# waveygang/wfmash

Measured on AMD Instinct MI355X. Metric: aligned bases/sec (whole node) + CIGAR-identical rate vs CPU ref, higher is better.
Workload: dtype int32; 1 GPU; C3: 64 synthetic 5%-divergence 50kb segment pairs per GPU, WFA-only (BiWFA gap-affine-2p 5,8,2,24,1; mappings pre-supplied); pairs_per_gpu=64, pairs_total=64, parallelism=records sharded over 1 GPU(s)

## Files before the change

include/wfmash_host.h:

```cpp
#ifndef WFMASH_HOST_H_
#define WFMASH_HOST_H_

#include <stdint.h>
#include "wfmash_hip.h"

#ifdef __cplusplus
extern "C" {
#endif

typedef struct {
  int32_t  mismatch, gap_open1, gap_ext1, gap_open2, gap_ext2;
  float    min_identity;
  uint64_t min_alignment_length;
  float    min_block_identity;
  uint64_t target_padding;
  uint64_t query_padding;
  uint64_t wflign_max_len_minor;
  int32_t  disable_chain_patching;
  int32_t  sam_format;
  int32_t  emit_md_tag;
  int32_t  no_seq_in_sam;
  int32_t  threads;
  int32_t  resident_sequences;
} wfmh_align_params_t;

typedef struct {
  uint64_t records;
  uint64_t aligned_bp;
  uint64_t written;
  uint64_t skipped;
  uint64_t cells;
  double   ms_gpu;
  double   ms_total;
  double   ms_rows;
  double   ms_fetch;
  double   ms_wflign;
  double   ms_text;
  uint64_t batches;
  uint64_t cells_tile;
  uint64_t tile_launches;
  double   ms_tile;
  double   ms_tags;
  uint64_t records_resident;
  uint64_t lazy_fetches;
} wfmh_align_summary_t;

void wfmh_align_default_params(wfmh_align_params_t* p);

int wfmh_align_paf(wfm_handle_t* h, const char* target_fasta, const char* query_fasta,
                   const char* mapping_paf, const char* out_paf,
                   const wfmh_align_params_t* params, wfmh_align_summary_t* summary);

int wfmh_align_paf_multi(wfm_handle_t* const* handles, int n, const char* target_fasta, const char* query_fasta,
                         const char* mapping_paf, const char* out_paf,
                         const wfmh_align_params_t* params, wfmh_align_summary_t* summary);

void wfmh_set_verify(int on);
int  wfmh_verify_counts(uint64_t out[4]);
int  wfmh_verify_paf(wfm_handle_t* h, const char* target_fasta, const char* query_fasta, const char* aligned_paf, uint64_t out[4]);
char* wfmh_test_verify_parse(const char* line);

void wfmh_set_verify_optimal(int on, uint64_t max_cells);
int  wfmh_verify_optimal_counts(uint64_t out[4]);

void wfmh_set_left_align(int on);
int  wfmh_left_align_counts(uint64_t out[4]);

void wfmh_set_cs(int form);
int  wfmh_cs_counts(uint64_t out[4]);

void wfmh_set_variants(const char* path_or_null);
int  wfmh_variants_counts(uint64_t out[4]);

void wfmh_set_coverage(const char* path_or_null);
int  wfmh_coverage_counts(uint64_t out[4]);
int  wfmh_coverage_paf(wfm_handle_t* h, const char* target_fasta, const char* aligned_paf, const char* out_path, uint64_t out[4]);
char* wfmh_test_coverage_bedgraph(const char* const* names, const uint64_t* lengths, int n_seq, const uint64_t* starts, const uint32_t* depths,
                                  int64_t n_iv);

void wfmh_set_lift(const char* bed_path_or_null, const char* out_path_or_null);
int  wfmh_lift_counts(uint64_t out[4]);
int  wfmh_lift_paf(wfm_handle_t* h, const char* target_fasta, const char* aligned_paf, const char* bed_path, const char* out_path, uint64_t out[4]);
void wfmh_set_chain(const char* path_or_null, int swap);
int  wfmh_chain_counts(uint64_t out[4]);
int  wfmh_chain_paf(wfm_handle_t* h, const char* target_fasta, const char* aligned_paf, const char* out_path, int swap, uint64_t out[4]);
void wfmh_set_maf(const char* path_or_null, uint32_t split);
int  wfmh_maf_counts(uint64_t out[4]);
int  wfmh_maf_paf(wfm_handle_t* h, const char* target_fasta, const char* query_fasta_or_null, const char* aligned_paf, const char* out_path, uint32_t split,
                  uint64_t out[4]);
char* wfmh_test_chain_lines(const char* spec, int swap, uint32_t* flags_out);
void wfmh_set_chain_net(const char* path_or_null);
int  wfmh_chain_net_counts(uint64_t out[4]);
int  wfmh_chain_net_paf(wfm_handle_t* h, const char* target_fasta, const char* aligned_paf, const char* out_path, uint64_t out[4]);
char* wfmh_test_chain_net_lines(const char* spec);
void wfmh_set_transitive(const char* bed_path_or_null, const char* out_path_or_null, uint32_t depth);
int  wfmh_transitive_counts(uint64_t out[4]);
int  wfmh_transitive_paf(wfm_handle_t* h, const char* target_fasta, const char* query_fasta_or_null, const char* aligned_paf, const char* bed_path,
                         const char* out_path, uint32_t depth, uint64_t out[4]);
char* wfmh_test_transitive_lines(const char* const* tnames, const uint64_t* tlengths, int n_t, const char* const* qnames, const uint64_t* qlengths,
                                 int n_q, const char* bed, const char* spec);

void wfmh_set_pav(const char* bed_path_or_null, uint64_t window, const char* out_path_or_null);
int  wfmh_pav_counts(uint64_t out[4]);
int  wfmh_pav_paf(wfm_handle_t* h, const char* target_fasta, const char* query_fasta_or_null, const char* aligned_paf, const char* bed_path_or_null,
                  uint64_t window, const char* out_path, uint64_t out[4]);
void wfmh_set_genotypes(const char* path_or_null);
int  wfmh_genotypes_counts(uint64_t out[4]);
char* wfmh_test_genotype_text(const char* version, const char* const* tnames, const uint64_t* lengths, int n_t, const char* const* keys, int n_groups,
                              const uint64_t* sites, size_t n_sites, const char* alleles, const char* gt);

char* wfmh_test_pav_text(const char* const* names, int n_q, const char* const* tnames, const uint64_t* lengths, int n_t, uint64_t window);

char* wfmh_test_lift_lines(const char* const* names, const uint64_t* lengths, int n_seq, const char* bed, const char* spec);

char* wfmh_test_cigar(const char* fn, const char* a, const char* b, const char* query, const char* target,
                      long long i0, long long i1);
void  wfmh_free(char* p);
void  wfmh_test_subwindow(int64_t win_start, int64_t win_end, int rev, int64_t a, int64_t b, int64_t* out_start, int64_t* out_end);
int wfmh_test_rows(const int32_t* q, int64_t n, int64_t* out);
int wfmh_test_tile_plan(const int32_t* jobs, int64_t n, const int32_t* rules, int32_t* per_block, int32_t* tasks, int64_t tasks_cap, int64_t* scalars);
int wfmh_test_p2_plan(const int32_t* cand, int64_t n, int64_t i0, int rows, int rows_bm, unsigned long long budget, int threads, int core, int64_t* geo,
                      int32_t* tasks, int64_t tasks_cap, int64_t* scalars);
int wfmh_test_base_plan(int op, const int32_t* in, int64_t n, int32_t* out);
int wfmh_test_reuse_plan(int op, const int64_t* in, int64_t n, int64_t* out);
int wfmh_test_planned_meet(const int64_t* in, int64_t n, int64_t* out);
int wfmh_test_tile_plan_dirs(const int32_t* jobs, int64_t n, const int32_t* rules, const uint8_t* dirs, int32_t* per_block, int32_t* tasks, int64_t tasks_cap,
                             int64_t* scalars);
int wfmh_test_tile_interior(const int32_t* q, int64_t n, int32_t* out);
int wfmh_test_tile_lean_waves(const int32_t* in, int64_t* out);
int wfmh_test_opt_band(const int64_t* in, int64_t* out);
int64_t wfmh_test_winnow(const char* seq, int64_t len, int k, int w, int s, int32_t seq_id,
                         const uint64_t* hash, const int8_t* strand, wfm_minmer_t* out, int64_t cap);

int64_t wfmh_test_winnow_chunked(const char* seq, int64_t len, int k, int w, int s, int32_t seq_id,
                                 const uint64_t* hash, const int8_t* strand, int64_t chunk_len,
                                 wfm_minmer_t* out, int64_t cap, int* replays);

int64_t wfmh_test_winnow_thinned(const char* seq, int64_t len, int k, int w, int s, int32_t seq_id,
                                 const uint64_t* hash, const int8_t* strand, double c_factor, int64_t chunk_len,
                                 wfm_minmer_t* out, int64_t cap, uint32_t* kept_pos, int64_t cap_kept,
                                 int64_t* n_kept, int* replays);

void wfmh_test_sort_records(wfm_minmer_t* recs, int64_t n, int threads);
int wfmh_test_packed_lce(const uint8_t* buf_p, int64_t n_p, int64_t start_p, const uint8_t* buf_t, int64_t n_t, int64_t start_t, int v, int h, int maxn);
int wfmh_test_is_acgt(const uint8_t* seq, int64_t n);

int64_t wfmh_test_winnow_model(const char* seq, int64_t len, int k, int w, int s, int32_t seq_id, const uint64_t* hash,
                               const int8_t* strand, double c_factor, int64_t chunk_len, wfm_minmer_t* out, int64_t cap,
                               uint32_t* why);

void wfmh_test_sortlike_model(wfm_minmer_t* recs, int64_t n);

int64_t wfmh_test_finish_records(const wfm_minmer_t* raw, int64_t n, int w, wfm_minmer_t* out, int64_t cap);


typedef struct {
  int32_t  kmer_size;
  int64_t  window_length;
  int64_t  block_length;
  int64_t  chain_gap;
  uint64_t max_mapping_length;
  float    percentage_identity;
  int32_t  sketch_size;
  int32_t  filter_mode;
  uint32_t num_mappings_for_segment;
  uint32_t num_mappings_for_scaffold;
  int32_t  drop_rand;
  int32_t  split;
  int32_t  merge_mappings;
  int32_t  skip_self;
  int32_t  skip_prefix;
  int32_t  lower_triangular;
  char     prefix_delim;
  int32_t  filter_length_mismatches;
  uint64_t sparsity_hash_threshold;
  double   overlap_threshold;
  double   scaffold_overlap_threshold;
  int64_t  scaffold_max_deviation;
  int64_t  scaffold_gap;
  int64_t  scaffold_min_length;
  int32_t  legacy_output;
  int32_t  minimum_hits;
  double   max_kmer_freq;
  int64_t  index_by_size;
  float    kmer_complexity_threshold;
  int32_t  stage1_topani_filter;
  int32_t  stage2_full_scan;
  float    ani_diff, ani_diff_conf;
  double   hg_numerator;
  int32_t  threads;
  int32_t  auto_pct_identity;
  int32_t  ani_percentile;
  float    ani_adjustment;
  const char* target_prefix;
  const char* target_list;
  const char* query_prefix;
  const char* query_list;
  const char* index_file;
  int32_t  write_index;
  int32_t  pad_;
  const char* scaffold_out;
  int32_t  streaming_minhash;
} wfmh_map_params_t;

void wfmh_map_default_params(wfmh_map_params_t* p);

typedef struct {
  uint64_t targets, queries, subsets;
  uint64_t target_bp, query_bp;
  uint64_t index_windows;
  uint64_t fragments;
  uint64_t l2_mappings;
  uint64_t written;
  float    percentage_identity;
  int32_t  sketch_size;
  double   ms_index, ms_map, ms_filter, ms_total;
  double   ms_replicate;
  double   ms_identity;
  double   ms_wall;
  int32_t  index_parts;
  int32_t  pad_;
  double   ms_index_sketch;
  double   ms_index_merge;
} wfmh_map_summary_t;

int wfmh_map(wfm_handle_t* h, const char* target_fasta, const char* query_fasta, const char* out_paf,
             const wfmh_map_params_t* params, wfmh_map_summary_t* summary);

int wfmh_map_multi(wfm_handle_t* const* handles, int n, const char* target_fasta, const char* query_fasta, const char* out_paf,
                   const wfmh_map_params_t* params, wfmh_map_summary_t* summary);

typedef struct {
  char*    query_group;
  char*    target_group;
  uint64_t query_hashes, target_hashes, shared;
  double   jaccard, ani;
} wfmh_ani_row_t;
int  wfmh_ani_matrix(wfm_handle_t* const* handles, int n, const char* target_fasta, const char* query_fasta,
                     const wfmh_map_params_t* params, const char* out_tsv);
int  wfmh_ani_matrix_rows(wfm_handle_t* const* handles, int n, const char* target_fasta, const char* query_fasta,
                          const wfmh_map_params_t* params, wfmh_ani_row_t** rows, int64_t* n_rows);
void wfmh_free_ani_rows(wfmh_ani_row_t* rows, int64_t n_rows);
void wfmh_set_ani_matrix(const char* out_tsv);
char* wfmh_test_ani_tsv(const char* const* query_groups, const char* const* target_groups, const uint64_t* query_hashes,
                        const uint64_t* target_hashes, const uint64_t* shared, int64_t n);

int wfmh_test_deal(const int64_t* lengths, int64_t n, int n_parts, int32_t* out_part);

int wfmh_test_map_plan(int op, const int64_t* in, int64_t n, int64_t* out);

int wfmh_seed_paf(const char* target_fasta, const char* query_fasta, const char* seeds_paf, const char* out_paf,
                  const wfmh_map_params_t* params, wfmh_map_summary_t* summary);

char* wfmh_test_filter(const char* stage, const wfm_mapping_t* maps, int64_t n, const char* fasta,
                       const char* query_name, const wfmh_map_params_t* prm);
char* wfmh_test_filter_ordered(const char* stage, const wfm_mapping_t* maps, int64_t n, const uint32_t* orig, const char* fasta,
                               const char* query_name, const wfmh_map_params_t* prm);

char* wfmh_test_fasta(const char* path, const char* name, int64_t start, int64_t end_inclusive, int whole);

void wfmh_release_sequences(void);

char* wfmh_test_fasta_shared(const char* path, const char* name);

int wfmh_test_index_file(const char* op, const char* fasta, char prefix_delim, const char* in_path, const char* out_path);

#ifdef __cplusplus
}
#endif
#endif
```

wfmash_amd/capi.py:

```python
import ctypes as C
import os

import numpy as np

_HERE = os.path.dirname(os.path.abspath(__file__))
LIB_PATH = os.environ.get("WFM_LIB_PATH") or os.path.join(_HERE, "libwfmash_hip.so")

WFM_MODE_END2END_BIWFA = 0
WFM_MODE_ENDSFREE = 1
WFM_MODE_END2END_UNI = 2
WFM_MODE_MASK = 0xff
WFM_MODE_SCORE_ONLY = 0x100
WFM_MODE_SCORE_LIMIT = 0x200
WFM_ST_MAX_SCORE = -100

DEFAULT_PEN = (5, 8, 2, 24, 1)
WFM_PF_ROOT_AGAIN, WFM_PF_JOB_AGAIN, WFM_PF_BASE_RETRY, WFM_PF_BASE_RETRY2, WFM_PF_BYTE_KERNEL, WFM_PF_P2_ROUNDS, WFM_PF_RING_KERNEL, WFM_PF_BASE_TILES = 1, 2, 4, 8, 16, 32, 64, 128
WFM_PF_RING_GROWN = 256
TILE_COUNTERS = ("jobs", "exact_ends", "fine_reruns", "gap_reruns", "ring3", "blocks_coarse", "blocks_fine", "left_band",
                 "reuse_resumed", "reuse_fallbacks", "reuse_keeps", "reuse_touched", "reuse_fell_other", "planned_ends",
                 "p2_exact", "p2_exact_misses")

EXPORTS = [
    "wfm_create", "wfm_destroy", "wfm_last_error", "wfm_device_name",
# ... 1566 lines not shown
        ident = np.ascontiguousarray(p2["ident_table"], dtype=np.uint16)
        cut = np.ascontiguousarray(p2["cutoff_j"], dtype=np.float64)
        P = MapParams()
        P.kmer_size = k
        P.kmer_complexity_threshold = kc_threshold
        P.l1 = L1Params(p1["window_length"], p1["sketch_size"], p1["min_hits_cached"], p1["cached_segment_length"],
                        int(p1["skip_self"]), int(p1["skip_prefix"]), int(p1["lower_triangular"]), int(p1["stage1_topani"]),
                        int(p1["stage2_full_scan"]), len(rg), rg.ctypes.data, mh.ctypes.data, sc.ctypes.data, len(sc), 0)
        P.l2 = L2Params(p2["window_length"], p2["sketch_size"], int(p2["stage1_topani"]), 0, keep.ctypes.data, ident.ctypes.data,
                        cut.ctypes.data)
        buf = np.frombuffer(seq, dtype=np.uint8)
        f = self._L.wfm_map_fragments
        f.restype = C.c_int64
        f.argtypes = [C.c_void_p, C.c_void_p, C.c_void_p, C.c_int64, C.c_void_p, C.c_void_p, C.c_int64, C.POINTER(MapParams),
                      C.c_void_p, C.c_void_p, C.c_int64]
        cap = 1 << 16
        while True:
            out = np.zeros(cap, dtype=MAPPING_DTYPE)
            frag = np.zeros(cap, dtype=np.int32)
            n = f(self._p, index._p, buf.ctypes.data, len(seq), off.ctypes.data, sid.ctypes.data, len(off), C.byref(P),
                  out.ctypes.data, frag.ctypes.data, cap)
            if n < 0:
                raise WfmError(f"wfm_map_fragments failed ({n}): {self.last_error()}")
            if n <= cap:
                return out[:n], frag[:n]
            cap = int(n)

    def minhash_sketch(self, seq: bytes, k: int = 21, sketch_size: int = 4096):
        out = np.zeros(sketch_size, dtype=np.uint64)
        buf = np.frombuffer(seq, dtype=np.uint8)
        f = self._L.wfm_minhash_sketch
        f.restype = C.c_int64
        f.argtypes = [C.c_void_p, C.c_void_p, C.c_int64, C.c_int, C.c_int, C.c_void_p]
        n = f(self._p, buf.ctypes.data, len(seq), k, sketch_size, out.ctypes.data)
        if n < 0:
            raise WfmError(f"wfm_minhash_sketch failed ({n}): {self.last_error()}")
        return out[:n]

    def sketch_intersections(self, sketches, rows=None, cols=None, offsets=None):
        n = len(sketches)
        parts = [np.ascontiguousarray(s, dtype=np.uint64) for s in sketches]
        hashes = np.concatenate(parts) if parts else np.zeros(0, dtype=np.uint64)
        if offsets is None:
            offsets = np.concatenate([[0], np.cumsum([len(p) for p in parts], dtype=np.int64)])
        offs = np.ascontiguousarray(offsets, dtype=np.int64)
        if len(offs) != n + 1:
            raise ValueError("one offset per sketch and one more")
        r = np.ascontiguousarray(np.arange(n) if rows is None else rows, dtype=np.int32)
        c = np.ascontiguousarray(np.arange(n) if cols is None else cols, dtype=np.int32)
        out = np.zeros((len(r), len(c)), dtype=np.uint32)
        f = self._L.wfm_sketch_intersections
        f.restype = C.c_int
        f.argtypes = [C.c_void_p, C.c_void_p, C.c_void_p, C.c_int64, C.c_void_p, C.c_int64, C.c_void_p, C.c_int64, C.c_void_p]
        rc = f(self._p, hashes.ctypes.data, offs.ctypes.data, n, r.ctypes.data, len(r), c.ctypes.data, len(c), out.ctypes.data)
        if rc != 0:
            raise WfmError(f"wfm_sketch_intersections failed ({rc}): {self.last_error()}")
        return out

    def map_l2(self, index, qsketch, qcount, q_len, q_kc, s, cands, params):
        nfrag = len(qcount)
        q = np.ascontiguousarray(qsketch, dtype=MINMER_DTYPE)
        qc = np.ascontiguousarray(qcount, dtype=np.int32)
        ql = np.ascontiguousarray(q_len, dtype=np.int32)
        kc = np.ascontiguousarray(q_kc, dtype=np.uint8)
        cd = np.ascontiguousarray(cands, dtype=L1_DTYPE)
        keep = np.ascontiguousarray(params["keep_table"], dtype=np.uint8)
        ident = np.ascontiguousarray(params["ident_table"], dtype=np.uint16)
        cut = np.ascontiguousarray(params["cutoff_j"], dtype=np.float64)
        S1 = params["sketch_size"] + 1
        assert keep.size == S1 * S1 and ident.size == S1 * S1 and cut.size == S1 and len(q) == nfrag * s
        P = L2Params(params["window_length"], params["sketch_size"], int(params["stage1_topani"]), 0, keep.ctypes.data,
                     ident.ctypes.data, cut.ctypes.data)
        f = self._L.wfm_map_l2
        f.restype = C.c_int64
        f.argtypes = [C.c_void_p, C.c_void_p, C.c_void_p, C.c_void_p, C.c_void_p, C.c_void_p, C.c_int64, C.c_int, C.c_void_p,
                      C.c_int64, C.POINTER(L2Params), C.c_void_p, C.c_void_p, C.c_int64]
        cap = 1 << 16
        while True:
            out = np.zeros(cap, dtype=MAPPING_DTYPE)
            frag = np.zeros(cap, dtype=np.int32)
            n = f(self._p, index._p, q.ctypes.data, qc.ctypes.data, ql.ctypes.data, kc.ctypes.data, nfrag, s, cd.ctypes.data, len(cd),
                  C.byref(P), out.ctypes.data, frag.ctypes.data, cap)
            if n < 0:
                raise WfmError(f"wfm_map_l2 failed ({n}): {self.last_error()}")
            if n <= cap:
                return out[:n], frag[:n]
            cap = int(n)

    def add_minmers_multi(self, seqs, k: int, w: int, s: int, seq_ids=None, threads: int = 1, cap=None):
        n = len(seqs)
        ids = np.ascontiguousarray(seq_ids if seq_ids is not None else range(n), dtype=np.int32)
        bufs = [np.frombuffer(x, dtype=np.uint8) for x in seqs]
        ptrs = (C.c_void_p * n)(*[b.ctypes.data for b in bufs])
        lens = np.array([len(x) for x in seqs], dtype=np.int64)
        cap = int(cap) if cap else 4 * int(lens.sum()) + 64
        out = np.zeros(cap, dtype=MINMER_DTYPE)
        counts = np.zeros(n, dtype=np.int64)
        f = self._L.wfm_add_minmers_multi
        f.restype = C.c_int64
        f.argtypes = [C.c_void_p, C.c_void_p, C.c_void_p, C.c_void_p, C.c_int64, C.c_int, C.c_int, C.c_int, C.c_int, C.c_void_p, C.c_int64,
                      C.c_void_p]
        tot = f(self._p, ptrs, lens.ctypes.data, ids.ctypes.data, n, k, w, s, threads, out.ctypes.data, cap, counts.ctypes.data)
        if tot < 0:
            raise WfmError(f"wfm_add_minmers_multi failed ({tot}): {self.last_error()}")
        offs = np.concatenate([[0], np.cumsum(counts)])
        return [out[offs[i]:offs[i + 1]] for i in range(n)]

    def finish_records(self, raw, w: int):
        raw = np.ascontiguousarray(raw, dtype=MINMER_DTYPE)
        f = self._L.wfm_finish_records
        f.restype = C.c_int64
        f.argtypes = [C.c_void_p, C.c_void_p, C.c_int64, C.c_int, C.c_void_p, C.c_int64, C.POINTER(C.c_int32), C.POINTER(C.c_int32)]
        cap = 4 * len(raw) + 64
        lv, hp = C.c_int32(0), C.c_int32(0)
        while True:
            out = np.zeros(cap, dtype=MINMER_DTYPE)
            n = f(self._p, raw.ctypes.data, len(raw), w, out.ctypes.data, cap, C.byref(lv), C.byref(hp))
            if n < 0:
                raise WfmError(f"wfm_finish_records failed ({n}): {self.last_error()}")
            if n <= cap:
                return out[:n], lv.value, hp.value
            cap = int(n)

    def prefilter_kmers(self, seq: bytes, k: int, w: int, s: int, c_factor: float = 4.0):
        cap = len(seq) + 1
        pos = np.zeros(cap, dtype=np.uint32)
        hsh = np.zeros(cap, dtype=np.uint64)
        st = np.zeros(cap, dtype=np.int8)
        buf = np.frombuffer(seq, dtype=np.uint8)
        f = self._L.wfm_prefilter_kmers
        f.restype = C.c_int64
        f.argtypes = [C.c_void_p, C.c_void_p, C.c_int64, C.c_int, C.c_int, C.c_int, C.c_double, C.c_void_p, C.c_void_p, C.c_void_p, C.c_int64]
        n = f(self._p, buf.ctypes.data, len(seq), k, w, s, c_factor, pos.ctypes.data, hsh.ctypes.data, st.ctypes.data, cap)
        if n < 0:
            raise WfmError(f"wfm_prefilter_kmers failed ({n}): {self.last_error()}")
        return pos[:n], hsh[:n], st[:n]

    def add_minmers(self, seq: bytes, k: int, w: int, s: int, seq_id: int = 0):
        cap = 4 * len(seq) + 64
        out = np.zeros(cap, dtype=MINMER_DTYPE)
        buf = np.frombuffer(seq, dtype=np.uint8)
        self._L.wfm_add_minmers.restype = C.c_int64
        self._L.wfm_add_minmers.argtypes = [C.c_void_p, C.c_void_p, C.c_int64, C.c_int, C.c_int, C.c_int, C.c_int32, C.c_void_p, C.c_int64]
        n = self._L.wfm_add_minmers(self._p, buf.ctypes.data, len(seq), k, w, s, seq_id, out.ctypes.data, cap)
        if n < 0:
            raise WfmError(f"wfm_add_minmers failed ({n}): {self.last_error()}")
        return out[:n]


HOST_EXPORTS = ["wfmh_test_packed_lce", "wfmh_test_is_acgt", "wfmh_align_default_params", "wfmh_align_paf", "wfmh_test_cigar", "wfmh_free", "wfmh_test_winnow",
                "wfmh_map_default_params", "wfmh_test_filter", "wfmh_map", "wfmh_test_winnow_chunked", "wfmh_test_fasta", "wfmh_test_winnow_thinned", "wfmh_test_sort_records", "wfmh_test_index_file",
                "wfmh_map_multi", "wfmh_align_paf_multi", "wfmh_test_winnow_model", "wfmh_test_sortlike_model", "wfmh_test_finish_records",
                "wfmh_release_sequences", "wfmh_test_fasta_shared", "wfmh_seed_paf", "wfmh_test_deal", "wfmh_test_subwindow",
                "wfmh_test_rows", "wfmh_test_tile_plan", "wfmh_test_p2_plan", "wfmh_test_base_plan", "wfmh_test_map_plan", "wfmh_test_filter_ordered",
                "wfmh_test_reuse_plan", "wfmh_test_planned_meet", "wfmh_test_tile_plan_dirs", "wfmh_test_tile_interior", "wfmh_test_tile_lean_waves", "wfmh_set_verify", "wfmh_verify_counts", "wfmh_verify_paf", "wfmh_test_verify_parse",
                "wfmh_set_verify_optimal", "wfmh_verify_optimal_counts", "wfmh_test_opt_band", "wfmh_set_left_align", "wfmh_left_align_counts", "wfmh_set_cs", "wfmh_cs_counts", "wfmh_set_variants", "wfmh_variants_counts",
                "wfmh_set_coverage", "wfmh_coverage_counts", "wfmh_coverage_paf", "wfmh_test_coverage_bedgraph",
                "wfmh_set_lift", "wfmh_lift_counts", "wfmh_lift_paf", "wfmh_test_lift_lines",
                "wfmh_set_chain", "wfmh_chain_counts", "wfmh_chain_paf", "wfmh_test_chain_lines",
                "wfmh_set_maf", "wfmh_maf_counts", "wfmh_maf_paf",
                "wfmh_set_chain_net", "wfmh_chain_net_counts", "wfmh_chain_net_paf", "wfmh_test_chain_net_lines",
                "wfmh_set_transitive", "wfmh_transitive_counts", "wfmh_transitive_paf", "wfmh_test_transitive_lines",
                "wfmh_set_pav", "wfmh_pav_counts", "wfmh_pav_paf", "wfmh_test_pav_text",
                "wfmh_set_genotypes", "wfmh_genotypes_counts", "wfmh_test_genotype_text",
                "wfmh_ani_matrix", "wfmh_ani_matrix_rows", "wfmh_free_ani_rows", "wfmh_set_ani_matrix", "wfmh_test_ani_tsv"]


class MapSummary(C.Structure):
    _fields_ = [("targets", C.c_uint64), ("queries", C.c_uint64), ("subsets", C.c_uint64), ("target_bp", C.c_uint64),
                ("query_bp", C.c_uint64), ("index_windows", C.c_uint64), ("fragments", C.c_uint64), ("l2_mappings", C.c_uint64),
                ("written", C.c_uint64), ("percentage_identity", C.c_float), ("sketch_size", C.c_int32), ("ms_index", C.c_double), ("ms_map", C.c_double), ("ms_filter", C.c_double),
                ("ms_total", C.c_double), ("ms_replicate", C.c_double), ("ms_identity", C.c_double), ("ms_wall", C.c_double),
                ("index_parts", C.c_int32), ("pad_", C.c_int32), ("ms_index_sketch", C.c_double), ("ms_index_merge", C.c_double)]


def _handle_array(handles):
    arr = (C.c_void_p * len(handles))(*[h._p for h in handles])
    return arr


def map_paf_multi(handles, target_fasta: str, out_paf: str, query_fasta: str = None, params=None) -> "MapSummary":
    L = load()
    L.wfmh_map_multi.restype = C.c_int
    L.wfmh_map_multi.argtypes = [C.c_void_p, C.c_int, C.c_char_p, C.c_char_p, C.c_char_p, C.c_void_p, C.POINTER(MapSummary)]
    s = MapSummary()
    rc = L.wfmh_map_multi(_handle_array(handles), len(handles), target_fasta.encode(), query_fasta.encode() if query_fasta else None,
                          out_paf.encode(), C.byref(params) if params is not None else None, C.byref(s))
    if rc != 0:
        raise WfmError(f"wfmh_map_multi failed ({rc}): {handles[0].last_error()}")
    return s


def seed_paf(target_fasta: str, seeds_paf: str, out_paf: str, query_fasta: str = None, params=None) -> "MapSummary":
    L = load()
    L.wfmh_seed_paf.restype = C.c_int
    L.wfmh_seed_paf.argtypes = [C.c_char_p, C.c_char_p, C.c_char_p, C.c_char_p, C.c_void_p, C.POINTER(MapSummary)]
    s = MapSummary()
    rc = L.wfmh_seed_paf(target_fasta.encode(), query_fasta.encode() if query_fasta else None, seeds_paf.encode(), out_paf.encode(),
                         C.byref(params) if params is not None else None, C.byref(s))
    if rc != 0:
        raise WfmError(f"wfmh_seed_paf failed ({rc})")
    return s


def map_paf(handle, target_fasta: str, out_paf: str, query_fasta: str = None, params=None) -> "MapSummary":
    L = load()
    L.wfmh_map.restype = C.c_int
    L.wfmh_map.argtypes = [C.c_void_p, C.c_char_p, C.c_char_p, C.c_char_p, C.c_void_p, C.POINTER(MapSummary)]
    s = MapSummary()
    rc = L.wfmh_map(handle._p, target_fasta.encode(), query_fasta.encode() if query_fasta else None, out_paf.encode(),
                    C.byref(params) if params is not None else None, C.byref(s))
    if rc != 0:
        raise WfmError(f"wfmh_map failed ({rc}): {handle.last_error()}")
    return s


class AniRowC(C.Structure):
    _fields_ = [("query_group", C.c_void_p), ("target_group", C.c_void_p), ("query_hashes", C.c_uint64), ("target_hashes", C.c_uint64),
                ("shared", C.c_uint64), ("jaccard", C.c_double), ("ani", C.c_double)]


def ani_matrix(handles_or_handle, target_fasta: str, query_fasta: str = None, params=None):
    L = load()
    handles = list(handles_or_handle) if isinstance(handles_or_handle, (list, tuple)) else [handles_or_handle]
    f = L.wfmh_ani_matrix_rows
    f.restype = C.c_int
    f.argtypes = [C.c_void_p, C.c_int, C.c_char_p, C.c_char_p, C.c_void_p, C.POINTER(C.POINTER(AniRowC)), C.POINTER(C.c_int64)]
    L.wfmh_free_ani_rows.restype = None
    L.wfmh_free_ani_rows.argtypes = [C.POINTER(AniRowC), C.c_int64]
    rows, n = C.POINTER(AniRowC)(), C.c_int64(0)
    rc = f(_handle_array(handles), len(handles), os.fsencode(target_fasta), os.fsencode(query_fasta) if query_fasta else None,
           C.byref(params) if params is not None else None, C.byref(rows), C.byref(n))
    if rc != 0:
        raise WfmError(f"wfmh_ani_matrix_rows failed ({rc}): {handles[0].last_error()}")
    try:
        return [(C.string_at(r.query_group).decode(), C.string_at(r.target_group).decode(), int(r.query_hashes), int(r.target_hashes),
                 int(r.shared), float(r.jaccard), float(r.ani)) for r in (rows[i] for i in range(n.value))]
    finally:
        L.wfmh_free_ani_rows(rows, n)


def ani_matrix_tsv(handles_or_handle, target_fasta: str, out_tsv: str, query_fasta: str = None, params=None) -> None:
    L = load()
    handles = list(handles_or_handle) if isinstance(handles_or_handle, (list, tuple)) else [handles_or_handle]
    f = L.wfmh_ani_matrix
    f.restype = C.c_int
    f.argtypes = [C.c_void_p, C.c_int, C.c_char_p, C.c_char_p, C.c_void_p, C.c_char_p]
    rc = f(_handle_array(handles), len(handles), os.fsencode(target_fasta), os.fsencode(query_fasta) if query_fasta else None,
           C.byref(params) if params is not None else None, os.fsencode(out_tsv))
    if rc != 0:
        raise WfmError(f"wfmh_ani_matrix failed ({rc}): {handles[0].last_error()}")


def set_ani_matrix(out_tsv) -> None:
    f = load().wfmh_set_ani_matrix
    f.restype = None
    f.argtypes = [C.c_char_p]
    f(os.fsencode(out_tsv) if out_tsv is not None else None)


def host_ani_tsv(rows) -> str:
    L = load()
    n = len(rows)
    enc = lambda x: x if isinstance(x, bytes) else x.encode()
    qn = (C.c_char_p * max(n, 1))(*[enc(r[0]) for r in rows])
    tn = (C.c_char_p * max(n, 1))(*[enc(r[1]) for r in rows])
    qh, th, sh = (np.array([r[j] for r in rows], dtype=np.uint64) for j in (2, 3, 4))
    f = L.wfmh_test_ani_tsv
    f.restype = C.c_void_p
    f.argtypes = [C.c_void_p, C.c_void_p, C.c_void_p, C.c_void_p, C.c_void_p, C.c_int64]
    L.wfmh_free.restype = None
    L.wfmh_free.argtypes = [C.c_void_p]
    p = f(qn, tn, qh.ctypes.data, th.ctypes.data, sh.ctypes.data, n)
    if not p:
        raise WfmError("wfmh_test_ani_tsv failed")
    s = C.string_at(p).decode()
    L.wfmh_free(p)
    return s


def host_deal(lengths, n_parts: int):
    L = load()
    L.wfmh_test_deal.restype = C.c_int
    L.wfmh_test_deal.argtypes = [C.c_void_p, C.c_int64, C.c_int, C.c_void_p]
    ln = np.ascontiguousarray(lengths, dtype=np.int64)
    out = np.zeros(max(len(ln), 1), dtype=np.int32)
    rc = L.wfmh_test_deal(ln.ctypes.data, len(ln), n_parts, out.ctypes.data)
    if rc != 0:
        raise WfmError(f"wfmh_test_deal failed ({rc})")
    return [int(x) for x in out[:len(ln)]]


def host_map_plan(op: int, values, out_size: int):
    L = load()
    L.wfmh_test_map_plan.restype = C.c_int
    L.wfmh_test_map_plan.argtypes = [C.c_int, C.c_void_p, C.c_int64, C.c_void_p]
    v = np.ascontiguousarray(values, dtype=np.int64)
    out = np.full(max(out_size, 1), -(1 << 62), dtype=np.int64)
    rc = L.wfmh_test_map_plan(op, v.ctypes.data, len(v), out.ctypes.data)
    if rc != 0:
        raise WfmError(f"wfmh_test_map_plan failed ({rc})")
    return out[:out_size]


def host_fasta_shared(path: str, name: str) -> str:
    L = load()
    L.wfmh_test_fasta_shared.restype = C.c_void_p
# ... 875 lines not shown
```

wfmash_amd/csrc/wfa_device.h:

```cpp
#ifndef WFM_WFA_DEVICE_H_
#define WFM_WFA_DEVICE_H_

#include <hip/hip_runtime.h>
#include <stdint.h>

#include "wfa_rows.h"

namespace wfm {

constexpr int WF_NULL = -(1 << 30);
constexpr int RING = 32;
constexpr int RMASK = RING - 1;
constexpr int RING_BIG = 128;

enum { C_M = 0, C_I1 = 1, C_I2 = 2, C_D1 = 3, C_D2 = 4 };
enum { OP_M = 0, OP_X = 1, OP_I = 2, OP_D = 3 };
enum { BT_I1_EXT = 8, BT_I2_EXT = 16, BT_D1_EXT = 32, BT_D2_EXT = 64 };

constexpr int WFM_DEV_UNREACHABLE = -300;
constexpr int WFM_DEV_OVERFLOW = -2;
constexpr int WFM_DEV_BAND = -4;
constexpr int WFM_DEV_P2_NOTHING = -6;
constexpr int WFM_DEV_LIMIT = -7;
constexpr int WFM_DEV_P2_MORE = -5;
// ... 229 lines not shown
  uint32_t n_runs, flags;
};
struct ChainWin {
  uint64_t count;
  uint32_t flags, lead_dt, lead_dq, trail_dt, trail_dq, eq, x, pad_;
};
void launch_chain_index(const uint32_t* runs, const ChainProb* probs, int nprob, void* pre, ChainWin* win, unsigned long long* off, hipStream_t st);
void launch_chain_write(const uint32_t* runs, const ChainProb* probs, const void* pre, const ChainWin* win, const unsigned long long* off, uint32_t ka,
                        uint32_t kb, void* out, hipStream_t st);
struct PavProb {
  uint64_t base, runs_off;
  uint32_t n_runs, group;
};
void launch_pav_count(const uint32_t* runs, const PavProb* probs, int nprob, unsigned long long n_bases, uint32_t n_groups, uint32_t* flags,
                      unsigned long long* cnt, unsigned long long* off, bool eq_only, hipStream_t st);
void launch_pav_write(const uint32_t* runs, const PavProb* probs, int nprob, const uint32_t* flags, const unsigned long long* off,
                      unsigned long long* ks, unsigned long long* ke, bool eq_only, hipStream_t st);
hipError_t pav_sort(void* tmp, size_t* tmp_bytes, const unsigned long long* ks, unsigned long long* ks2, const unsigned long long* ke,
                    unsigned long long* ke2, unsigned long long n, unsigned end_bit, hipStream_t st);
void launch_pav_runmax(unsigned long long* ke, unsigned long long n, unsigned long long* aux, hipStream_t st);
void launch_pav_compact(const unsigned long long* ks, const unsigned long long* rm, unsigned long long n, unsigned long long* aux,
                        unsigned long long* uks, unsigned long long* uke, hipStream_t st);
void launch_pav_prefix(const unsigned long long* uks, const unsigned long long* uke, unsigned long long m, unsigned long long* aux,
                       unsigned long long* C, hipStream_t st);
void launch_pav_matrix(const unsigned long long* uks, const unsigned long long* uke, const unsigned long long* C, unsigned long long m, const void* iv,
                       unsigned long long ra, unsigned long long rb, uint32_t n_groups, uint32_t* out, hipStream_t st);
struct SiteVar {
  uint64_t pos;
  uint32_t kind, group;
  uint32_t ref_len, alt_len;
  uint64_t off;
};
struct SiteRow {
  uint64_t pos;
  uint32_t kind, n_carrier_groups;
  uint32_t ref_len, alt_len;
  uint64_t off;
};
struct SitesWork {
  unsigned long long *k1, *k2, *kg, *ks;
  uint32_t *k3, *sk3, *pa, *pb;
  uint32_t *first, *gfirst;
  uint8_t* flag;
  const unsigned long long* tasks;
  unsigned long long* aux;
};
void launch_sites_fold(uint8_t* alle, unsigned long long bytes, hipStream_t st);
void launch_sites_keys(const SiteVar* vars, const uint8_t* alle, uint32_t n, const SitesWork& w, unsigned long long n_tasks, unsigned hash_bits, hipStream_t st);
void launch_sites_gather64(const unsigned long long* in, const uint32_t* perm, uint32_t n, unsigned long long* out, hipStream_t st);
void launch_sites_gather32(const uint32_t* in, const uint32_t* perm, uint32_t n, uint32_t* out, hipStream_t st);
hipError_t sites_sort64(void* tmp, size_t* tmp_bytes, const unsigned long long* k, unsigned long long* k2, const uint32_t* v, uint32_t* v2, uint32_t n,
                        unsigned end_bit, hipStream_t st);
hipError_t sites_sort32(void* tmp, size_t* tmp_bytes, const uint32_t* k, uint32_t* k2, const uint32_t* v, uint32_t* v2, uint32_t n, unsigned end_bit,
                        hipStream_t st);
void launch_sites_heads(const SiteVar* vars, const uint8_t* alle, uint32_t n, const SitesWork& w, const uint32_t* perm, uint32_t* inv,
                        unsigned long long n_tasks, hipStream_t st);
void launch_sites_rows(const SiteVar* vars, const uint32_t* perm, const uint32_t* first, const uint32_t* gfirst, uint32_t n_sites, SiteRow* rows, hipStream_t st);
void launch_sites_gt(const SiteRow* rows, const uint32_t* first, const uint32_t* sk3, const unsigned long long* uks, const unsigned long long* uke,
                     const unsigned long long* C, unsigned long long m, unsigned long long ra, unsigned long long rb, uint32_t n_groups, uint8_t* out,
                     hipStream_t st);
struct NetProb {
  uint64_t base, runs_off;
  uint32_t n_runs, score;
  uint64_t order;
};
struct NetBlock {
  uint64_t order, t;
  uint32_t q, size;
};
struct NetRec {
  uint64_t order;
  uint32_t score, zero;
};
struct NetPer {
  uint64_t order;
  uint32_t score, zero;
  uint64_t first, count, won, aligned;
};
void launch_net_count(const uint32_t* runs, const NetProb* probs, int nprob, unsigned long long n_bases, uint32_t* flags, unsigned long long* word,
                      unsigned long long* off, uint32_t* score, hipStream_t st);
void launch_net_write(const uint32_t* runs, const NetProb* probs, int nprob, const uint32_t* flags, const unsigned long long* off, const uint32_t* score,
                      NetBlock* blocks, NetRec* recs, hipStream_t st);
struct NetWork {
  const NetBlock* blocks; unsigned long long n;
  const NetRec* recs; uint32_t r;
  unsigned long long *e, *e2;
  unsigned long long* aux;
  uint32_t* brank;
  unsigned long long *ro, *so;
  uint32_t *ri, *sp;
  unsigned long long *k2, *k2s;
  uint32_t *p2, *prio, *sscore;
  unsigned long long *aligned, *won;
  uint32_t* bad;
  unsigned long long* tree;
  unsigned long long m;
  unsigned long long *ps, *pe, *pw;
  uint32_t *key, *val, *sk, *sv;
  unsigned long long p;
};
void launch_net_ends(const NetWork& w, hipStream_t st);
hipError_t net_sort_keys(void* tmp, size_t* tmp_bytes, const unsigned long long* k, unsigned long long* k2, unsigned long long n, unsigned end_bit, hipStream_t st);
void launch_net_distinct(const NetWork& w, hipStream_t st);
void launch_net_rec_keys(const NetWork& w, hipStream_t st);
void launch_net_rec_rank(const NetWork& w, hipStream_t st);
void launch_net_prio(const NetWork& w, hipStream_t st);
void launch_net_fill(const NetWork& w, hipStream_t st);
void launch_net_push(const NetWork& w, hipStream_t st);
void launch_net_heads_count(const NetWork& w, hipStream_t st);
void launch_net_heads_write(const NetWork& w, hipStream_t st);
void launch_net_piece_keys(const NetWork& w, hipStream_t st);
void launch_net_pieces(const NetWork& w, unsigned long long a, unsigned long long b, NetBlock* out, hipStream_t st);
void launch_net_per(const NetWork& w, NetPer* per, hipStream_t st);
struct TransProb {
  uint64_t t, q, runs_off;
  uint32_t n_runs, flags;
};
struct TransSpan {
  uint32_t flags, pspan, tspan, pad_;
};
struct TransArc {
  uint64_t s, d, pre;
  uint32_t slen, n_runs;
};
constexpr uint64_t TRANS_ARC_BACK = (uint64_t)1 << 62, TRANS_ARC_REVERSE = (uint64_t)1 << 63, TRANS_ARC_PRE = TRANS_ARC_BACK - 1;
void launch_trans_span(const uint32_t* runs, const TransProb* probs, int nprob, unsigned long long n_bases, TransSpan* out, hipStream_t st);
void launch_trans_pre(const uint32_t* runs, const TransProb* probs, int nprob, const unsigned long long* pre_off, void* pre, hipStream_t st);
void launch_trans_keys(const TransArc* arcs, unsigned long long n, unsigned long long* key, unsigned long long* idx, hipStream_t st);
void launch_trans_index(const TransArc* arcs, const unsigned long long* idx, unsigned long long n, TransArc* sorted, unsigned long long* maxs,
                        unsigned long long* pm, hipStream_t st);
void launch_trans_count(const unsigned long long* ks, const unsigned long long* ke, unsigned long long m, const unsigned long long* pks,
                        const unsigned long long* pke, unsigned long long m_prev, const TransArc* arcs, const unsigned long long* pm,
                        unsigned long long n_arcs, void* win, unsigned long long* cnt, unsigned long long* off, hipStream_t st);
void launch_trans_write(const unsigned long long* ks, const unsigned long long* ke, const void* win, const unsigned long long* off,
                        unsigned long long ka, unsigned long long kb, const TransArc* arcs, const void* pre, unsigned long long* oks,
                        unsigned long long* oke, hipStream_t st);
struct OptProb {
  int64_t p_off, t_off, row_off;
  int32_t plen, tlen;
  int32_t pbf, pef, tbf, tef;
  int32_t band_lo, band_hi;
};
void launch_optcheck(const uint8_t* seq, const OptProb* probs, int nprob, int form, int32_t* rows, int32_t* out, DevPen pen, hipStream_t st);
void launch_seq_normalize(uint8_t* seq, int64_t nbytes, hipStream_t st);
void launch_seq_pack(const uint8_t* seq, uint32_t* pk, int64_t nwords, int64_t nbytes, const SeqRev* jobs, int njobs, int32_t* flag, hipStream_t st);
constexpr int64_t PK_PAD_WORDS = 2048 + 64;
void launch_tile2(const uint32_t* pk, int32_t* ring, const TileJob* jobs, const TileTask* tasks, int32_t* mak, int ntasks, int threads, int T, int variants, hipStream_t st);
#ifndef WFM_TILE_SLOTS_WIDE
#define WFM_TILE_SLOTS_WIDE 16
#endif
constexpr int TILE_SLOTS_WAVE1 = 2, TILE_SLOTS_SMALL = 4, TILE_SLOTS_WIDE = WFM_TILE_SLOTS_WIDE;
constexpr int tile_fine_slots(int threads) { return threads <= 64 ? TILE_SLOTS_WAVE1 : (threads <= 128 ? TILE_SLOTS_SMALL : TILE_SLOTS_WIDE); }
bool tile2_coarse_maxima();
void launch_tile2_p2(const uint32_t* pk, int32_t* ring, const TileJob* jobs, const TileTask* tasks, int ntasks, int threads, int32_t* p2, hipStream_t st);
int selftest_dpp(int* host_out128, hipStream_t st);
void launch_base2(const uint32_t* pk, int32_t* a32, uint8_t* a8, uint32_t* rle, const BaseJob* jobs, BaseResult* res, int njobs, int threads, hipStream_t st);
void launch_bp(const uint8_t* seq, int32_t* ring, const BpJob* jobs, BpResult* res, int njobs, int threads,
               DevPen pen, int scope, int ring_rows, hipStream_t st);
void launch_tile_init(const uint8_t* seq, int32_t* ring, const TileJob* jobs, int32_t* mak0, int njobs, int ring_rows, hipStream_t st);
void launch_tile(const uint8_t* seq, int32_t* ring, const TileJob* jobs, const TileTask* tasks, int32_t* mak, int ntasks,
                 int threads, int T, int Wt, size_t lds_bytes, DevPen pen, int scope, int ring_rows, hipStream_t st);
void launch_tile_advance(TileJob* jobs, int32_t* mak, int njobs, int T, DevPen pen, int exact, int coarse, int launched, hipStream_t st);
void launch_tile_reg(const uint8_t* seq, int32_t* ring, const TileJob* jobs, const TileTask* tasks, int32_t* mak, int ntasks,
                     int threads, int T, int C, bool cut, hipStream_t st);
void launch_tile_p2(const uint8_t* seq, int32_t* ring, const TileJob* jobs, const TileTask* tasks, int ntasks, int threads,
                    int32_t* p2, bool cut, hipStream_t st);
void launch_p2_to_ring(int32_t* ring, const int32_t* p2, const P2Job* jobs, int njobs, hipStream_t st);
struct RingWidenJob {
  const int32_t* src;
  int32_t* dst;
  int32_t src_w, src_koff;
  int32_t dst_w, dst_koff;
  int32_t klo, khi;
};
void launch_ring_widen(const RingWidenJob* jobs, int njobs, int max_dst_w, int ring_rows, hipStream_t st);
void launch_p2_blockmax(const int32_t* ring, const int32_t* p2, const P2Job* jobs, int32_t* bmax, int32_t* p2max, int njobs, hipStream_t st);
void launch_p2_overlap(const int32_t* ring, const int32_t* p2, const P2Job* jobs, const int32_t* p2max, const int32_t* bmax,
                       BpResult* res, int njobs, int threads, int max_nblk, DevPen pen, int scope, hipStream_t st);
void launch_p2_exact(const int32_t* ring, const int32_t* p2, const P2Job* jobs, BpResult* res, int njobs, int threads, DevPen pen, int scope, hipStream_t st);
void launch_base(const uint8_t* seq, int32_t* a32, uint8_t* a8, uint32_t* rle, const BaseJob* jobs, BaseResult* res,
                 int njobs, DevPen pen, bool wide, int ring_rows, hipStream_t st);
void launch_compact(const uint32_t* rle, const int64_t* off, const int64_t* cap, uint32_t* out, unsigned long long* total,
                    int64_t* out_start, int32_t* out_count, int nprob, hipStream_t st);

}
#endif
```

wfmash_amd/csrc/wfa_host.hip:

```cpp
#include <hip/hip_runtime.h>

#include <algorithm>
#include <chrono>
#include <climits>
#include <cstdio>
#include <cstring>
#include <atomic>
#include <mutex>
#include <string>
#include <thread>
#include <vector>

#include "../../include/wfmash_hip.h"
#include "wfa_host_shared.h"
#include "wfa_plan.h"
#include "wfa_optband.h"

#ifdef WFM_PROFILE_SECTIONS
namespace wfm { void read_sections(long long* out); }
#endif
namespace wfm { void p2_counters(unsigned long long* out); }
namespace {

using namespace wfm;
// ... 714 lines not shown
  const int rc = launch_keeps(p);
  if (rc != WFM_OK) return rc;
  HIPCHK(h, hipMemcpyAsync(p.got.data(), h->tilejobs.p, p.n * sizeof(TileJob), hipMemcpyDeviceToHost, h->stream));
  return WFM_OK;
}

int time_chunk(TilePhase& p) {
  wfm_handle* h = p.h;
  const size_t ntasks = p.plan.tasks.size();
  for (int b = 0; b < p.chunk; ++b) {
    float ms = 0;
    HIPCHK(h, hipEventElapsedTime(&ms, h->tile_ev[2 * b], h->tile_ev[2 * b + 1]));
    p.tile_ms += ms;
    if (h->call_base) {
      float t0 = 0;
      HIPCHK(h, hipEventElapsedTime(&t0, h->call_base, h->tile_ev[2 * b]));
      h->tile_iv.emplace_back(t0, t0 + ms);
    }
  }
  p.blocks += (uint32_t)p.chunk;
  for (int b = 0; b < p.chunk; ++b) p.lane_cells += (double)ntasks * p.plan.threads_b[(size_t)b] * p.cfg.C * p.T;
  h->stats.tile_launches += (uint32_t)p.chunk;
  h->stats.tile_tasks += (uint32_t)(ntasks * (size_t)p.chunk);
  return WFM_OK;
}

void account_chunk(TilePhase& p) {
  wfm_handle* h = p.h;
  const int T = p.T;
  p.n_active = 0;
  for (size_t i = 0; i < p.n; ++i) {
    const TileJob& was = p.tj[i];
    const TileJob& got = p.got[i];
    for (int bl = was.nblocks; bl < got.nblocks; ++bl) {
      const bool last_exact = got.mode == 2 && bl == got.nblocks - 1;
      const int base = p.s_begin[i] + ((last_exact && got.plan_sum <= 0) ? bl - 1 : bl) * T;
      for (int d = 0; d < 2; ++d) {
        if (!((p.dirs[i] >> d) & 1)) continue;
        const int steps = last_exact ? (d == 0 ? got.tf : got.tr) : T;
        p.tile_cells += (uint64_t)cells_sum(was.pl, was.tl, was.sub, base + 1, base + steps);
      }
    }
    if (got.fine_s == -1 && was.fine_s != -1) {
      for (int d = 0; d < 2; ++d) if ((p.dirs[i] >> d) & 1) p.tile_cells += (uint64_t)cells_sum(was.pl, was.tl, was.sub, got.s0 + 1, got.s0 + T);
      h->tile_ctr[WFM_TC_FINE_RERUNS] += 1;
      p.reruns5 += 1;
    }
    if (got.reran > was.reran) {
      for (int d = 0; d < 2; ++d) if ((p.dirs[i] >> d) & 1) p.tile_cells += (uint64_t)cells_sum(was.pl, was.tl, was.sub, got.s0 - T + 1, got.s0);
      h->tile_ctr[WFM_TC_GAP_RERUNS] += (uint64_t)(got.reran - was.reran);
      p.reruns6 += (uint32_t)(got.reran - was.reran);
    }
    p.tj[i] = got;
    p.active[i] = (char)(got.active != 0);
    p.fmax[i] = got.fmax; p.rmax[i] = got.rmax;
    p.n_active += p.active[i];
  }
}

void hand_back(TilePhase& p, uint32_t level, double cells_before) {
  wfm_handle* h = p.h;
  uint64_t unique_level = 0;
  for (size_t i = 0; i < p.n; ++i) {
    const TileJob& t = p.tj[i];
    const int sf_end = t.mode == 2 ? t.s0 + t.tf : t.s0, sr_end = t.mode == 2 ? t.s0 + t.tr : t.s0;
    if (p.ru && p.ru->bad[i]) continue;
    unique_level += (uint64_t)cells_sum(t.pl, t.tl, t.sub, p.s_begin[i] + 1, sf_end) + (uint64_t)cells_sum(t.pl, t.tl, t.sub, p.s_begin[i] + 1, sr_end);
  }
  h->stats.cells_tile_unique += unique_level;
  for (size_t i = 0; i < p.n; ++i) {
    const TileJob& t = p.tj[i];
    BpJob& j = p.jobs[(size_t)p.tiled[i]];
    j.ring_off = t.ring_in;
    p.ring2[i] = t.ring_out;
    j.resume_s = t.s0;
    j.resume_sr = -1; j.last_fwd = 0;
    h->tile_ctr[WFM_TC_EXACT_ENDS] += t.mode == 2;
    h->tile_ctr[WFM_TC_PLANNED_ENDS] += t.mode == 2 && t.plan_sum > 0;
    h->tile_ctr[WFM_TC_LEFT_BAND] += t.mode == 3 && !(p.ru && p.ru->bad[i]);
    if (t.mode == 3) {
      j.resume_s = -3; j.resume_sr = t.s0; j.fmax0 = p.fmax[i]; j.rmax0 = p.rmax[i];
      continue;
    }
    if (t.mode == 2) {
      j.resume_s = t.s0 + t.tf;
      j.resume_sr = t.s0 + t.tr;
      j.last_fwd = t.last_fwd;
    }
    j.fmax0 = p.fmax[i]; j.rmax0 = p.rmax[i];
  }
  if (p.cfg.debug) fprintf(stderr, "[wfm] level %u: tiled %zu jobs, %u blocks of %d scores (Wt %d), %.3f ms; %.3e cells computed on %.3e lane-steps (%.0f %% of the lanes hold a cell), %.3e of them in the result (the block in which a job's wavefronts meet runs twice); launches of the packed kernel without / with per-score maxima %u / %u, mode-5 reruns %u, mode-6 reruns %u\n", level, p.n, p.blocks, p.T, p.cfg.Wt, p.tile_ms,
                           (double)p.tile_cells - cells_before, p.lane_cells, p.lane_cells > 0 ? 100.0 * ((double)p.tile_cells - cells_before) / p.lane_cells : 0.0, (double)unique_level,
                           p.launches_coarse, p.launches_fine, p.reruns5, p.reruns6);
}

int run_tiled_phase(wfm_handle* h, wfm_seqset* S, const DevPen& dp, int scope, const TileCfg& cfg, int T, bool refine,
                    std::vector<BpJob>& jobs, const std::vector<int>& tiled, std::vector<int64_t>& ring2,
                    double& tile_ms, uint64_t& tile_cells, uint32_t level, const std::vector<int32_t>* fine_from = nullptr,
                    const std::vector<int64_t>* ring3 = nullptr, ReuseCtl* reuse = nullptr, const std::vector<int32_t>* plan_from = nullptr) {
  const size_t n = tiled.size();
  if (n == 0) return WFM_OK;
  const double cells_before = (double)tile_cells;
  TilePhase p{h, S, dp, scope, cfg, T, refine, jobs, tiled, ring2, tile_ms, tile_cells, n};
  p.ru = refine ? nullptr : reuse;
  int rc = init_tile_jobs(p, fine_from, ring3, plan_from);
  if (rc != WFM_OK) return rc;
  if (p.n_active) {
    HIPCHK(h, hipMemcpyAsync(h->tilejobs.p, p.tj.data(), n * sizeof(TileJob), hipMemcpyHostToDevice, h->stream));
    HIPCHK(h, hipMemsetAsync(h->tilemak.p, 0, n * 2 * (size_t)T * sizeof(int32_t), h->stream));
    p.chunk = std::max(1, std::min(cfg.chunk, (int)h->tile_ev.size() / 2));
    p.got.resize(n); p.pjobs.resize(n);
    p.rules = TilePlanRules{cfg.threads, cfg.C, T, p.chunk, cfg.Wt - 2 * T, cfg.reg, cfg.fine, cfg.reg && cfg.exact && tile2_coarse_maxima(), p.any_planned};
    auto clk = [] { return std::chrono::steady_clock::now(); };
    auto msd = [](std::chrono::steady_clock::time_point a, std::chrono::steady_clock::time_point b) { return std::chrono::duration<double, std::milli>(b - a).count(); };
    double ms_prep = 0, ms_launch = 0, ms_wait = 0, ms_post = 0;
    while (p.n_active) {
      const auto tq0 = clk();
      if ((rc = drop_leavers(p)) != WFM_OK) return rc;
      if (!p.n_active) break;
      if ((rc = plan_tile_tasks(p)) != WFM_OK) return rc;
      const auto tq1 = clk();
      if ((rc = launch_chunk(p)) != WFM_OK) return rc;
      const auto tq2 = clk();
      HIPCHK(h, hipStreamSynchronize(h->stream));
      const auto tq3 = clk();
      if ((rc = time_chunk(p)) != WFM_OK) return rc;
      account_chunk(p);
      settle_keeps(p);
      if ((rc = restore_kept(p)) != WFM_OK) return rc;
      ms_prep += msd(tq0, tq1); ms_launch += msd(tq1, tq2); ms_wait += msd(tq2, tq3); ms_post += msd(tq3, clk());
    }
    if (cfg.debug > 1)
      fprintf(stderr, "[wfm] level %u tile phase, host side: task lists %.2f ms, launches %.2f ms, waiting for the device %.2f ms, bookkeeping %.2f ms\n", level, ms_prep, ms_launch, ms_wait, ms_post);
  }
  hand_back(p, level, cells_before);
  return WFM_OK;
}


struct P2Chunk {
  wfm_handle* h; wfm_seqset* S; const DevPen& dp; int scope; const TileCfg& cfg; std::vector<BpJob>& jobs;
  const std::vector<int>& cand; const std::vector<int64_t>& ring_other; std::vector<BpResult>& res; double& ms_out;
  std::vector<BpResult>& carry; std::vector<char>& has_carry; bool may_continue; std::vector<int>& again;
  const std::vector<int32_t>& exact_of;
  std::vector<P2PlanJob> pcand;
  std::vector<char> pexact;
  P2ChunkPlan plan;
  size_t i0 = 0, n = 0;
  std::vector<TileJob> tj;
  std::vector<P2Job> pj;
  std::vector<int> at;
  std::vector<P2Job> pj_dev;
  size_t ns = 0, ns_dump = 0;
  std::vector<BpResult> got;
  float ms = 0;
};

void fill_p2_chunk(P2Chunk& c, size_t i0) {
  const size_t budget = std::max<size_t>(c.h->mem_budget / 4, (size_t)64 << 20);
  plan_p2_chunk(c.pcand.data(), c.pcand.size(), i0, P2K, P2ROWS, budget, c.cfg.threads, c.cfg.Wt - 2 * P2K, c.plan, c.pexact.data());
  c.i0 = i0; c.n = c.plan.geo.size();
  c.tj.clear(); c.pj.clear();
  c.at.assign(c.n, 0); c.ns = 0;
  for (size_t q = 0; q < c.n; ++q) c.ns += !c.pexact[i0 + q];
  for (size_t q = 0, s = 0, e = c.ns; q < c.n; ++q) c.at[q] = (int)(c.pexact[i0 + q] ? e++ : s++);
  for (size_t q = 0; q < c.n; ++q) {
    const BpJob& j = c.jobs[(size_t)c.cand[i0 + q]];
    const P2Geometry& g = c.plan.geo[q];
    TileJob t = tile_job_from(j);
    t.ring_out = c.ring_other[i0 + q];
    t.mode = 4; t.tf = j.resume_s; t.tr = j.resume_sr; t.last_fwd = j.last_fwd;
    t.p2_off = (int64_t)g.p2_off; t.w2 = (int32_t)g.w2; t.koff2 = g.koff2;
    P2Job pq{};
    pq.ring_in = j.ring_off; pq.p2_off = (int64_t)g.p2_off; pq.width = j.width; pq.koff = j.koff; pq.w2 = (int32_t)g.w2; pq.koff2 = g.koff2;
    pq.pl = j.pl; pq.tl = j.tl; pq.sf = j.resume_s; pq.sr = j.resume_sr; pq.last_fwd = j.last_fwd; pq.sub = j.sub; pq.best0 = j.best0;
    pq.nblk = (int32_t)g.nblk; pq.bm_off = (int64_t)g.bm_off; pq.exact = c.exact_of[i0 + q];
    c.tj.push_back(t); c.pj.push_back(pq);
  }
  c.pj_dev.resize(c.n);
  for (size_t q = 0; q < c.n; ++q) c.pj_dev[(size_t)c.at[q]] = c.pj[q];
}

int launch_p2_chunk(P2Chunk& c) {
  wfm_handle* h = c.h;
  wfm_seqset* S = c.S;
  const size_t n = c.n, ns = c.ns, elems = c.plan.elems, bm_elems = c.plan.bm_elems, n_pk = c.plan.tiles.n_pk;
  const std::vector<TileTask>& tasks = c.plan.tiles.tasks;
  const int threads_c = c.plan.threads_c;
  if (h->p2rows.ensure(elems + 16) || h->p2max.ensure(ns * 2 * P2ROWS * 5) || h->p2bmax.ensure(bm_elems + 16) ||
      h->p2jobs.ensure(n) || h->tilejobs.ensure(n) || h->tiletasks.ensure(tasks.size()) || h->bpres.ensure(std::max(n, c.jobs.size()))) {
    h->err = "out of device memory (phase-2 rows)"; return WFM_E_NOMEM;
  }
  HIPCHK(h, hipMemcpyAsync(h->tilejobs.p, c.tj.data(), n * sizeof(TileJob), hipMemcpyHostToDevice, h->stream));
  HIPCHK(h, hipMemcpyAsync(h->p2jobs.p, c.pj_dev.data(), n * sizeof(P2Job), hipMemcpyHostToDevice, h->stream));
  HIPCHK(h, hipMemcpyAsync(h->tiletasks.p, tasks.data(), tasks.size() * sizeof(TileTask), hipMemcpyHostToDevice, h->stream));
  HIPCHK(h, hipEventRecord(h->ev0, h->stream));
  bool any_cut = false;
  for (const TileJob& t : c.tj) any_cut |= t.sub != SUB_NONE;
  if (n_pk) launch_tile2_p2(S->d_pk, h->ring.p, h->tilejobs.p, h->tiletasks.p, (int)n_pk, threads_c, h->p2rows.p, h->stream);
  if (tasks.size() > n_pk) launch_tile_p2(S->d_seq, h->ring.p, h->tilejobs.p, h->tiletasks.p + n_pk, (int)(tasks.size() - n_pk), threads_c, h->p2rows.p, any_cut, h->stream);
  static const int p2_threads = getenv("WFM_P2_THREADS") ? atoi(getenv("WFM_P2_THREADS")) : 0;
  static const int p2x_threads = getenv("WFM_P2_EXACT_THREADS") ? atoi(getenv("WFM_P2_EXACT_THREADS")) : 0;
  auto launch_search = [&](size_t cnt) {
    launch_p2_blockmax(h->ring.p, h->p2rows.p, h->p2jobs.p, h->p2bmax.p, h->p2max.p, (int)cnt, h->stream);
    launch_p2_overlap(h->ring.p, h->p2rows.p, h->p2jobs.p, h->p2max.p, h->p2bmax.p, h->bpres.p, (int)cnt,
                      p2_threads > 0 ? p2_threads : 1024, (int)(c.plan.maxw2 >> 6) + 1, c.dp, c.scope, h->stream);
  };
  if (ns) launch_search(ns);
  launch_p2_exact(h->ring.p, h->p2rows.p, h->p2jobs.p + ns, h->bpres.p + ns, (int)(n - ns), p2x_threads > 0 ? p2x_threads : p2_exact_threads(c.plan.maxw2), c.dp, c.scope, h->stream);
  HIPCHK(h, hipGetLastError());
  HIPCHK(h, hipEventRecord(h->ev1, h->stream));
  std::vector<BpResult> dev(n);
  HIPCHK(h, hipMemcpyAsync(dev.data(), h->bpres.p, n * sizeof(BpResult), hipMemcpyDeviceToHost, h->stream));
  HIPCHK(h, hipStreamSynchronize(h->stream));
  HIPCHK(h, hipEventElapsedTime(&c.ms, h->ev0, h->ev1));
  auto note_busy = [&](float ms) {
    if (!h->call_base) return hipSuccess;
    float t0 = 0;
    const hipError_t e = hipEventElapsedTime(&t0, h->call_base, h->ev0);
    if (e == hipSuccess) h->bp_iv.emplace_back(t0, t0 + ms);
    return e;
  };
  HIPCHK(h, note_busy(c.ms));
  c.got.resize(n);
  for (size_t q = 0; q < n; ++q) c.got[q] = dev[(size_t)c.at[q]];
  c.ns_dump = ns;
  h->tile_ctr[WFM_TC_P2_EXACT] += n - ns;
  std::vector<size_t> miss;
  for (size_t q = 0; q < n; ++q) if (c.got[q].status == WFM_DEV_P2_EXACT_MISS) miss.push_back(q);
  if (!miss.empty()) {
    h->tile_ctr[WFM_TC_P2_EXACT_MISSES] += miss.size();
    std::vector<P2Job> mj;
    size_t bm = 0;
    for (size_t q : miss) {
      P2Job& pq = c.pj[q];
      pq.exact = 0; pq.bm_off = (int64_t)bm;
      bm += (size_t)pq.nblk * 2 * P2ROWS * 5;
      mj.push_back(pq);
    }
    if (h->p2max.ensure(mj.size() * 2 * P2ROWS * 5) || h->p2bmax.ensure(bm + 16)) { h->err = "out of device memory (phase-2 maxima)"; return WFM_E_NOMEM; }
    HIPCHK(h, hipMemcpyAsync(h->p2jobs.p, mj.data(), mj.size() * sizeof(P2Job), hipMemcpyHostToDevice, h->stream));
    HIPCHK(h, hipEventRecord(h->ev0, h->stream));
    launch_search(mj.size());
    HIPCHK(h, hipGetLastError());
    HIPCHK(h, hipEventRecord(h->ev1, h->stream));
    HIPCHK(h, hipMemcpyAsync(dev.data(), h->bpres.p, mj.size() * sizeof(BpResult), hipMemcpyDeviceToHost, h->stream));
    HIPCHK(h, hipStreamSynchronize(h->stream));
    float ms2 = 0;
    HIPCHK(h, hipEventElapsedTime(&ms2, h->ev0, h->ev1));
    HIPCHK(h, note_busy(ms2));
    c.ms += ms2;
    for (size_t m = 0; m < miss.size(); ++m) c.got[miss[m]] = dev[m];
    c.ns_dump = 0;
  }
  c.ms_out += c.ms;
  return WFM_OK;
}

int dump_p2_job(P2Chunk& c) {
  wfm_handle* h = c.h;
  const std::vector<BpResult>& got = c.got;
  if (c.ns_dump == 0) { fprintf(stderr, "[wfm] p2 dump: no job of this chunk of %zu searches with its row maxima at hand (%zu take the exact walk)\n", c.n, c.n - c.ns); return WFM_OK; }
  const size_t pos = std::min<size_t>((size_t)c.cfg.p2_dump, c.ns_dump - 1);
  size_t q = 0;
  while ((size_t)c.at[q] != pos) ++q;
  std::vector<int32_t> rm((size_t)2 * P2ROWS * 5);
  HIPCHK(h, hipMemcpy(rm.data(), h->p2max.p + pos * 2 * P2ROWS * 5, rm.size() * 4, hipMemcpyDeviceToHost));
  const P2Job& pjq = c.pj[q];
  fprintf(stderr, "[wfm] p2 dump job %zu: pl %d tl %d sf %d sr %d last_fwd %d sub %d w2 %d nblk %d -> status %d score %d (fwd %d rev %d comp %d k %d) rounds %d\n", q, pjq.pl, pjq.tl, pjq.sf,
          pjq.sr, pjq.last_fwd, pjq.sub, pjq.w2, pjq.nblk, got[q].status, got[q].score, got[q].score_fwd, got[q].score_rev, got[q].comp, got[q].k_fwd, got[q].pad_);
  for (int d = 0; d < 2; ++d)
    for (int r = 0; r < P2ROWS; r += 3) {
      const int32_t* m = rm.data() + ((size_t)d * P2ROWS + r) * 5;
      fprintf(stderr, "[wfm]   dir %d row %d (s = %d): max M %d I1 %d I2 %d D1 %d D2 %d\n", d, r, (d == 0 ? pjq.sf : pjq.sr) - RNG_BACK + r, m[0], m[1], m[2], m[3], m[4]);
    }
  return WFM_OK;
}

void print_p2_chunk(const P2Chunk& c) {
  const std::vector<BpResult>& got = c.got;
  const std::vector<P2Job>& pj = c.pj;
  const size_t n = c.n;
  int more = 0;
  double tk = 0, tc = 0, rd = 0; uint32_t tkmax = 0; int rdmax = 0;
  for (const BpResult& r : got) { more += r.status == WFM_DEV_P2_MORE; tk += r.ticks_p2; tc += r.ticks_p1; rd += r.pad_; tkmax = std::max(tkmax, r.ticks_p2); rdmax = std::max(rdmax, r.pad_); }
  double tests = 0; int tests_max = 0;
  for (const BpResult& r : got) { tests += r.steps - r.steps_p1; tests_max = std::max(tests_max, r.steps - r.steps_p1); }
  size_t missed = 0;
  for (size_t q = 0; q < n; ++q) missed += pj[q].exact == 0 && (size_t)c.at[q] >= c.ns;
  fprintf(stderr, "[wfm] phase 2 from rows computed ahead: %zu jobs, widest %zu columns, %zu tiles of %d threads, %.3f ms, %d left to the step kernel; walk per job: %.1f rounds (max %d), %.0f us (max %.0f), of which cells stage %.0f us; "
          "%.1f tests (max %d); exact walk %.1f %% of the jobs, missed %.1f %%\n",
          n, c.plan.maxw2, c.plan.tiles.tasks.size(), c.plan.threads_c, c.ms, more, rd / n, rdmax, tk / n / 100.0, tkmax / 100.0, tc / n / 100.0, tests / n, tests_max,
          100.0 * (n - c.ns) / n, 100.0 * missed / n);
  size_t qs = 0;
  for (size_t q = 0; q < n; ++q) if (got[q].ticks_p2 > got[qs].ticks_p2) qs = q;
  fprintf(stderr, "[wfm]   slowest walk: pl %d tl %d sub %d w2 %d nblk %d: %d rounds, %.0f us = listing %.0f + cells %.0f (incl. listing) + pick %.0f, %u blocks listed, status %d\n", pj[qs].pl, pj[qs].tl,
          pj[qs].sub == SUB_NONE ? -1 : pj[qs].sub, pj[qs].w2, pj[qs].nblk, got[qs].pad_, got[qs].ticks_p2 / 100.0, got[qs].ticks_list / 100.0, got[qs].ticks_p1 / 100.0, got[qs].ticks_pick / 100.0,
          got[qs].work_items, got[qs].status);
}

int continue_p2_chunk(P2Chunk& c) {
  wfm_handle* h = c.h;
  std::vector<BpResult>& got = c.got;
  std::vector<P2Job> mj;
  for (size_t q = 0; q < c.n; ++q) {
    const size_t jq = (size_t)c.cand[c.i0 + q];
    BpJob& j = c.jobs[jq];
    if (got[q].status == WFM_DEV_P2_NOTHING) { got[q] = c.carry[jq]; continue; }
    if (got[q].status != WFM_DEV_P2_MORE) continue;
    if (got[q].comp >= 0) {
      c.carry[jq] = got[q]; c.carry[jq].status = 0; c.has_carry[jq] = 1;
      j.best0 = got[q].score;
    }
    if (!c.may_continue || (j.band > 0 && std::max(j.resume_s, j.resume_sr) + 2 * P2K + 2 > j.band)) continue;
    mj.push_back(c.pj[q]);
    j.resume_s += P2K; j.resume_sr += P2K;
    c.again.push_back((int)(c.i0 + q));
  }
  if (!mj.empty()) {
    HIPCHK(h, hipMemcpyAsync(h->p2jobs.p, mj.data(), mj.size() * sizeof(P2Job), hipMemcpyHostToDevice, h->stream));
    launch_p2_to_ring(h->ring.p, h->p2rows.p, h->p2jobs.p, (int)mj.size(), h->stream);
    HIPCHK(h, hipGetLastError());
    HIPCHK(h, hipStreamSynchronize(h->stream));
  }
  for (size_t q = 0; q < c.n; ++q) c.res[(size_t)c.cand[c.i0 + q]] = got[q];
  return WFM_OK;
}

int run_p2_phase(wfm_handle* h, wfm_seqset* S, const DevPen& dp, int scope, const TileCfg& cfg, std::vector<BpJob>& jobs,
                 const std::vector<int>& cand, const std::vector<int64_t>& ring_other, std::vector<BpResult>& res, double& ms_out,
                 std::vector<BpResult>& carry, std::vector<char>& has_carry, bool may_continue, std::vector<int>& again, const std::vector<int32_t>& exact_of) {
  if (cand.empty()) return WFM_OK;
  P2Chunk c{h, S, dp, scope, cfg, jobs, cand, ring_other, res, ms_out, carry, has_carry, may_continue, again, exact_of};
  for (size_t i = 0; i < cand.size(); ++i) {
    const BpJob& j = jobs[(size_t)cand[i]];
    c.pcand.push_back(P2PlanJob{j.pl, j.tl, j.sub, j.resume_s, j.resume_sr, j.packed});
    c.pexact.push_back((char)(exact_of[i] > 0));
  }
  for (size_t i0 = 0; i0 < cand.size(); i0 += c.n) {
    fill_p2_chunk(c, i0);
    int rc = launch_p2_chunk(c);
    if (rc != WFM_OK) return rc;
    if (cfg.p2_dump_on && (rc = dump_p2_job(c)) != WFM_OK) return rc;
    h->stats.p2_launches++;
    h->stats.p2_jobs += (uint32_t)c.n;
    if (cfg.debug) print_p2_chunk(c);
    if ((rc = continue_p2_chunk(c)) != WFM_OK) return rc;
  }
  return WFM_OK;
}


struct Knobs {
  static int num(const char* name, int dflt) { const char* e = getenv(name); return e ? atoi(e) : dflt; }
  bool use_hints = num("WFM_SCORE_HINT", 1) != 0;
  bool use_bound = use_hints && num("WFM_BOUND", 1) != 0;
  int slack_env = num("WFM_SUB_SLACK", -1);
  bool ring3_on = num("WFM_TILE_RING3", 1) != 0, p2_on = num("WFM_P2", 1) != 0;
  bool p2_exact = num("WFM_P2_EXACT", 1) != 0;
  int p2_rounds = std::max(1, num("WFM_P2_ROUNDS", 64));
  int fine_margin = num("WFM_TILE_FINE_MARGIN", 48);
  int coarse_min_blocks = num("WFM_TILE_COARSE_MIN_BLOCKS", 32), coarse_max_jobs = num("WFM_TILE_COARSE_MAX_JOBS", 128);
  bool planned_end = num("WFM_TILE_PLANNED_END", 1) != 0 && slack_env < (1 << 28);
  bool tile_v2 = num("WFM_TILE_V2", 1) != 0;
  bool band_on = num("WFM_BAND", 1) != 0;
  int band_root = std::max(64, num("WFM_BAND_ROOT", 4096));
  int resume_margin = num("WFM_RESUME_MARGIN", SNAP_ROWS);
  bool reuse = num("WFM_REUSE", 1) != 0 && slack_env < (1 << 28);
  int reuse_min_blocks = std::max(1, num("WFM_REUSE_MIN_BLOCKS", 8));
  int reuse_every = std::max(1, num("WFM_REUSE_EVERY", 2)), reuse_slack = std::max(0, num("WFM_REUSE_TOUCH_SLACK", 0));
  int reuse_levels = num("WFM_REUSE_LEVELS", 8);
  int debug = env_debug();
};

struct Chunk {
  std::vector<BpJob> jobs;
  std::vector<int32_t> node_of;
  size_t ring_elems = 0, end = 0;
  int maxw = 0;
  std::vector<int> tiled, tiled_r;
  std::vector<int64_t> ring2, ring3, ring2_r;
  std::vector<int32_t> fine_from, fine_r, snap_r;
  std::vector<int32_t> plan_from;
  std::vector<size_t> ring_third;
  std::vector<char> grown_job, resume_bad, has_carry;
  std::vector<ReuseUse> reuse;
  std::vector<int32_t> keep_upto;
  std::vector<char> reuse_bad;
  std::vector<std::vector<int32_t>> kept[2];
  std::vector<BpResult> res, carry;
  std::vector<int> rest, more_set;
  void clear() {
    jobs.clear(); node_of.clear(); ring_elems = 0; maxw = 0;
    tiled.clear(); ring2.clear(); ring3.clear(); ring_third.clear(); fine_from.clear();
    tiled_r.clear(); ring2_r.clear(); fine_r.clear(); snap_r.clear(); grown_job.clear();
    reuse.clear(); keep_upto.clear(); plan_from.clear();
  }
};

struct AlignCall {
  wfm_handle* h;
  const wfm_penalties_t* pen;
  wfm_seqset* S;
  size_t first, last;
  wfm_result_t* out;
  char* ops_arena;
  size_t arena_bytes, arena_base;
  std::vector<uint32_t>* runs_out;
  uint32_t* pflags;
  int scope;
  DevPen dp;
  const Knobs knobs;
  TileCfg tcfg;
  BaseCfg bcfg;
  int RR;
  RingRules rules;
  std::vector<int32_t> prob_status;
  std::vector<uint64_t> prob_cells;
  std::vector<int32_t> prob_score;
  std::vector<Node> bp_nodes, base_nodes, next_bp;
  uint32_t level = 0;
  Chunk ck;
  LevelTimer tm;
  double wall_tile = 0, wall_base = 0;
  uint64_t band_retries = 0, band_jobs = 0, roots_banded = 0, roots_out = 0, hint_retries = 0, limit_out = 0;
  uint64_t grown_jobs = 0, grown_widened = 0, grown_restarts = 0;
  int64_t grown_maxband = 0;
  size_t ring_peak = 0;
  GrownSnaps snaps;
  KeepStore keeps;
  uint64_t reuse_children = 0, reuse_found = 0, reuse_taken = 0;
  uint64_t keep_bytes = 0, restore_bytes = 0;
  uint64_t reuse_full_rings = 0;
};

void make_roots(AlignCall& c) {
  for (size_t i = c.first; i < c.last; ++i) {
    const ProbMeta& pm = c.S->meta[i];
    Node nd{};
    nd.prob = (int32_t)i; nd.pb = 0; nd.pl = pm.plen; nd.tb = 0; nd.tl = pm.tlen;
    nd.cb = C_M; nd.ce = C_M; nd.score_rem = INT_MAX; nd.endsfree = 0;
    nd.sub = SUB_NONE; nd.hinted = 0;
    if (c.pflags && (pm.mode == WFM_MODE_END2END_BIWFA || pm.mode == WFM_MODE_ENDSFREE) && !((size_t)i < c.S->acgt.size() && c.S->acgt[i])) c.pflags[i] |= WFM_PF_BYTE_KERNEL;
    if (c.knobs.use_hints && pm.hint > 0 && pm.mode == WFM_MODE_END2END_BIWFA) { nd.sub = pm.hint; nd.hinted = 1; }
    if (pm.limit > 0) { nd.limit = pm.limit; nd.sub = pm.limit; nd.hinted = 1; }
    int64_t bound = (int64_t)gapcost(*c.pen, pm.plen) + gapcost(*c.pen, pm.tlen) + 8;
    if (pm.limit > 0 && (pm.plen == 0 || pm.tlen == 0) && bound - 8 > pm.limit) { c.prob_status[i] = WFM_ST_MAX_SCORE; continue; }
    if (pm.limit > 0) bound = std::min<int64_t>(bound, pm.limit);
    if (pm.mode == WFM_MODE_ENDSFREE) {
      nd.endsfree = 1;
      nd.smax = (int32_t)std::min<int64_t>(bound, 256);
      c.base_nodes.push_back(nd);
    } else if (pm.mode == WFM_MODE_END2END_UNI || std::max(pm.plen, pm.tlen) <= BIALIGN_FALLBACK_MIN_LENGTH ||
               pm.plen == 0 || pm.tlen == 0) {
      nd.smax = (int32_t)std::min<int64_t>(bound, 256);
      c.base_nodes.push_back(nd);
    } else {
      c.bp_nodes.push_back(nd);
    }
  }
}

int bound_roots(AlignCall& c) {
  wfm_handle* h = c.h;
  std::vector<BoundJob> bj;
  std::vector<size_t> owner;
  if (c.knobs.use_bound)
    for (size_t q = 0; q < c.bp_nodes.size(); ++q) {
      const Node& nd = c.bp_nodes[q];
      const ProbMeta& pm = c.S->meta[nd.prob];
      if (pm.mode != WFM_MODE_END2END_BIWFA || std::min(nd.pl, nd.tl) < 1024 || std::abs(nd.tl - nd.pl) < 64) continue;
      bj.push_back(BoundJob{pm.p_fwd, pm.t_fwd, nd.pl, nd.tl});
      owner.push_back(q);
    }
  if (bj.empty()) return WFM_OK;
  uint64_t bounded_roots = 0, bound_gain = 0;
  const auto tb0 = std::chrono::steady_clock::now();
  if (h->bndjobs.ensure(bj.size()) || h->bndres.ensure(bj.size())) { h->err = "out of device memory (score bounds)"; return WFM_E_NOMEM; }
  HIPCHK(h, hipMemcpyAsync(h->bndjobs.p, bj.data(), bj.size() * sizeof(BoundJob), hipMemcpyHostToDevice, h->stream));
  launch_bound(c.S->d_seq, h->bndjobs.p, h->bndres.p, (int)bj.size(), c.dp, h->stream);
  HIPCHK(h, hipGetLastError());
  std::vector<int32_t> ub(bj.size());
  HIPCHK(h, hipMemcpyAsync(ub.data(), h->bndres.p, bj.size() * sizeof(int32_t), hipMemcpyDeviceToHost, h->stream));
  HIPCHK(h, hipStreamSynchronize(h->stream));
  for (size_t q = 0; q < bj.size(); ++q) {
    if (ub[q] < 0) continue;
// ... 1415 lines not shown
```

wfmash_amd/csrc/wfa_kernels.hip:

```cpp
#include <hip/hip_runtime.h>
#include <stdint.h>
#include <algorithm>
#include <cstdlib>
#include <type_traits>

#include "wfa_device.h"
#include "wfa_base.h"

namespace wfm {

#ifdef WFM_PROFILE_SECTIONS
__device__ long long g_sec[8];
#define SEC_T(v) const long long v = clock64(); asm volatile("" ::: "memory")
#define SEC_ADD(i, a, b) sec[i] += (b) - (a)
#else
#define SEC_T(v)
#define SEC_ADD(i, a, b)
#endif

__device__ __forceinline__ uint64_t load8(const uint8_t* p) {
  uint64_t v;
  __builtin_memcpy(&v, p, 8);
  return v;
}
// ... 1271 lines not shown
      score += key >> 8;
      v += rdlane(dv, w); h += rdlane(dh, w);
      forced = 0;
    } else {
      if (++forced > 6) { give_up(); return; }
      score += pen.x; ++v; ++h;
    }
  }
  score += gap(pl - v) + gap(tl - h);
  if (lane == 0) out[i] = score < (long long)(SUB_NONE - 1) ? (int32_t)score : -1;
}
void launch_bound(const uint8_t* seq, const BoundJob* jobs, int32_t* out, int njobs, DevPen pen, hipStream_t st) {
  hipLaunchKernelGGL(wfa_bound_kernel, dim3(njobs), dim3(64), 0, st, seq, jobs, out, pen, njobs);
}

__global__ __launch_bounds__(256) void seq_reverse_kernel(uint8_t* __restrict__ seq, const SeqRev* __restrict__ jobs, int pad) {
  const SeqRev J = jobs[blockIdx.x >> 1];
  const bool text = blockIdx.x & 1;
  const uint8_t* src = seq + (text ? J.t_fwd : J.p_fwd);
  uint8_t* dst = seq + (text ? J.t_rev : J.p_rev);
  const int n = text ? J.tlen : J.plen;
  for (int q = threadIdx.x; q < n + pad; q += blockDim.x) dst[q] = q < n ? src[n - 1 - q] : (uint8_t)0;
}
void launch_reverse(uint8_t* seq, const SeqRev* jobs, int njobs, int pad, hipStream_t st) {
  hipLaunchKernelGGL(seq_reverse_kernel, dim3(njobs * 2), dim3(256), 0, st, seq, jobs, pad);
}

namespace {
__device__ __forceinline__ uint32_t gather_complement4(uint32_t w) {
  const uint32_t b1 = (w >> 1) & 0x01010101u, b3 = (w >> 3) & 0x01010101u;
  const uint32_t cg = b1 & ~b3, at = ~b1 & ~b3 & 0x01010101u & (w >> 6);
  return w ^ (cg << 2) ^ (at | (at << 2) | (at << 4));
}
__device__ __forceinline__ uint32_t gather_pick(const uint32_t (&w)[8], int k) {
  uint32_t v = w[0];
#pragma unroll
  for (int j = 1; j < 8; ++j) v = k == j ? w[j] : v;
  return v;
}
}
__global__ __launch_bounds__(256) void seq_gather_kernel(const SeqGatherTask* __restrict__ tasks) {
  const SeqGatherTask T = tasks[blockIdx.x];
  const int64_t n = (int64_t)T.len + T.pad;
  const uintptr_t d = (uintptr_t)T.dst, s = (uintptr_t)T.src, s_end = s + (uintptr_t)T.len;
  const uintptr_t d0 = d & ~(uintptr_t)15;
  const int64_t nslots = (int64_t)((d + (uintptr_t)n + 15 - d0) >> 4);
  for (int64_t j = threadIdx.x; j < nslots; j += blockDim.x) {
    const uintptr_t D = d0 + ((uintptr_t)j << 4);
    const int64_t qb = (int64_t)D - (int64_t)d;
    uint32_t o[4] = {0u, 0u, 0u, 0u};
    if (qb < T.len) {
      const int64_t A = T.reverse ? (int64_t)s_end - 16 - qb : (int64_t)s + qb;
      const int64_t A0 = A & ~(int64_t)15;
      const int sh = (int)(A & 15);
      uint32_t w[8];
#pragma unroll
      for (int half = 0; half < 2; ++half) {
        const int64_t W = A0 + 16 * half;
        uint4 q = make_uint4(0u, 0u, 0u, 0u);
        if (W < (int64_t)s_end && W + 16 > (int64_t)s && (half == 0 || sh != 0)) q = *reinterpret_cast<const uint4*>((uintptr_t)W);
        w[4 * half] = q.x; w[4 * half + 1] = q.y; w[4 * half + 2] = q.z; w[4 * half + 3] = q.w;
      }
      uint32_t v[4];
#pragma unroll
      for (int i = 0; i < 4; ++i) {
        const int k = (sh >> 2) + i;
        const uint32_t lo = gather_pick(w, k), hi = k + 1 < 8 ? gather_pick(w, k + 1) : 0u;
        v[i] = __builtin_amdgcn_alignbyte(hi, lo, (uint32_t)(sh & 3));
      }
      if (T.reverse) {
#pragma unroll
        for (int i = 0; i < 4; ++i) o[i] = __builtin_amdgcn_perm(0u, v[3 - i], 0x00010203u);
      } else {
#pragma unroll
        for (int i = 0; i < 4; ++i) o[i] = v[i];
      }
      if (T.complement) {
#pragma unroll
        for (int i = 0; i < 4; ++i) o[i] = gather_complement4(o[i]);
      }
    }
    if (qb >= 0 && qb + 16 <= T.len) {
      *reinterpret_cast<uint4*>(D) = make_uint4(o[0], o[1], o[2], o[3]);
    } else {
      uint8_t* dst = reinterpret_cast<uint8_t*>(D);
#pragma unroll
      for (int b = 0; b < 16; ++b) {
        const int64_t q = qb + b;
        if (q >= 0 && q < n) dst[b] = q < T.len ? (uint8_t)(o[b >> 2] >> (8 * (b & 3))) : (uint8_t)0;
      }
    }
  }
}
void launch_seq_gather(const SeqGatherTask* tasks, int64_t ntasks, hipStream_t st) {
  if (ntasks > 0) hipLaunchKernelGGL(seq_gather_kernel, dim3((unsigned)ntasks), dim3(256), 0, st, tasks);
}

__global__ __launch_bounds__(256) void seq_normalize_kernel(uint8_t* __restrict__ seq, int64_t nwords) {
  const int64_t i = (int64_t)blockIdx.x * blockDim.x + threadIdx.x;
  if (i >= nwords) return;
  uint4 q = *reinterpret_cast<const uint4*>(seq + i * 16);
  uint32_t w[4] = {q.x, q.y, q.z, q.w};
#pragma unroll
  for (int j = 0; j < 4; ++j) {
    uint32_t out = 0;
#pragma unroll
    for (int b = 0; b < 4; ++b) {
      uint32_t c = (w[j] >> (8 * b)) & 0xffu;
      if (c > 96u && c < 123u) c -= 32u;
      if (!(c == 'A' || c == 'C' || c == 'G' || c == 'T')) c = 'N';
      out |= c << (8 * b);
    }
    w[j] = out;
  }
  *reinterpret_cast<uint4*>(seq + i * 16) = make_uint4(w[0], w[1], w[2], w[3]);
}
void launch_seq_normalize(uint8_t* seq, int64_t nbytes, hipStream_t st) {
  const int64_t nwords = (nbytes + 15) / 16;
  if (nwords > 0) hipLaunchKernelGGL(seq_normalize_kernel, dim3((unsigned)((nwords + 255) / 256)), dim3(256), 0, st, seq, nwords);
}

#ifdef WFM_PROFILE_SECTIONS
void read_sections(long long* out) { (void)hipMemcpyFromSymbol(out, HIP_SYMBOL(g_sec), sizeof(long long) * 8); }
#endif
void launch_bp(const uint8_t* seq, int32_t* ring, const BpJob* jobs, BpResult* res, int njobs, int threads,
               DevPen pen, int scope, int ring_rows, hipStream_t st) {
  if (ring_rows == RING) hipLaunchKernelGGL(r32::wfa_bp_kernel, dim3(njobs), dim3(threads), 0, st, seq, ring, jobs, res, pen, scope);
  else hipLaunchKernelGGL(r128::wfa_bp_kernel, dim3(njobs), dim3(threads), 0, st, seq, ring, jobs, res, pen, scope);
}
void launch_tile_init(const uint8_t* seq, int32_t* ring, const TileJob* jobs, int32_t* mak0, int njobs, int ring_rows, hipStream_t st) {
  if (ring_rows == RING) hipLaunchKernelGGL(r32::wfa_tile_init_kernel, dim3(njobs * 2), dim3(64), 0, st, seq, ring, jobs, mak0, njobs);
  else hipLaunchKernelGGL(r128::wfa_tile_init_kernel, dim3(njobs * 2), dim3(64), 0, st, seq, ring, jobs, mak0, njobs);
}
void launch_tile(const uint8_t* seq, int32_t* ring, const TileJob* jobs, const TileTask* tasks, int32_t* mak, int ntasks,
                 int threads, int T, int Wt, size_t lds_bytes, DevPen pen, int scope, int ring_rows, hipStream_t st) {
  if (ring_rows == RING) {
    (void)hipFuncSetAttribute((const void*)r32::wfa_tile_kernel, hipFuncAttributeMaxDynamicSharedMemorySize, (int)lds_bytes);
    hipLaunchKernelGGL(r32::wfa_tile_kernel, dim3(ntasks), dim3(threads), lds_bytes, st, seq, ring, jobs, tasks, mak, T, Wt, pen, scope);
  } else {
    (void)hipFuncSetAttribute((const void*)r128::wfa_tile_kernel, hipFuncAttributeMaxDynamicSharedMemorySize, (int)lds_bytes);
    hipLaunchKernelGGL(r128::wfa_tile_kernel, dim3(ntasks), dim3(threads), lds_bytes, st, seq, ring, jobs, tasks, mak, T, Wt, pen, scope);
  }
}
void launch_tile_advance(TileJob* jobs, int32_t* mak, int njobs, int T, DevPen pen, int exact, int coarse, int launched, hipStream_t st) {
  hipLaunchKernelGGL(wfa_tile_advance_kernel, dim3(njobs), dim3(64), 0, st, jobs, mak, njobs, T, pen, exact, coarse, launched);
}
void launch_tile_reg(const uint8_t* seq, int32_t* ring, const TileJob* jobs, const TileTask* tasks, int32_t* mak, int ntasks,
                     int threads, int T, int C, bool cut, hipStream_t st) {
  const size_t lds = (size_t)(T + 1) * 4;
  if (C == 4) hipLaunchKernelGGL((wfa_tile_reg_kernel<4, 256, 5, 10, 25, 2, 1>), dim3(ntasks), dim3(threads), lds, st, seq, ring, jobs, tasks, mak, T);
  else if (cut) hipLaunchKernelGGL((wfa_tile_reg_kernel<2, 1024, 5, 10, 25, 2, 1, false, true>), dim3(ntasks), dim3(threads), lds, st, seq, ring, jobs, tasks, mak, T);
  else hipLaunchKernelGGL((wfa_tile_reg_kernel<2, 1024, 5, 10, 25, 2, 1, false, false>), dim3(ntasks), dim3(threads), lds, st, seq, ring, jobs, tasks, mak, T);
}
void launch_tile_p2(const uint8_t* seq, int32_t* ring, const TileJob* jobs, const TileTask* tasks, int ntasks, int threads,
                    int32_t* p2, bool cut, hipStream_t st) {
  const size_t lds = (size_t)(P2K + 1) * 4;
  if (cut) hipLaunchKernelGGL((wfa_tile_reg_kernel<2, 1024, 5, 10, 25, 2, 1, true, true>), dim3(ntasks), dim3(threads), lds, st, seq, ring, jobs, tasks,
                              (int32_t*)nullptr, P2K, p2, (int32_t*)nullptr);
  else hipLaunchKernelGGL((wfa_tile_reg_kernel<2, 1024, 5, 10, 25, 2, 1, true, false>), dim3(ntasks), dim3(threads), lds, st, seq, ring, jobs, tasks,
                          (int32_t*)nullptr, P2K, p2, (int32_t*)nullptr);
}
__global__ __launch_bounds__(256) void wfa_p2_to_ring_kernel(int32_t* __restrict__ ring, const int32_t* __restrict__ p2, const P2Job* __restrict__ jobs) {
  const int job = blockIdx.x / (2 * 5 * RING), rest = blockIdx.x % (2 * 5 * RING), d = rest / (5 * RING), cc = (rest / RING) % 5, r = rest % RING;
  const P2Job J = jobs[job];
  const int sd = d == 0 ? J.sf : J.sr, s = sd + P2K - r;
  const Rng RG = make_rng(J.pl, J.tl, J.sub);
  const int lo = rng_lo(RG, s), hi = rng_hi(RG, s);
  const int32_t* src = p2 + J.p2_off + J.koff2 + ((int64_t)((d * 5 + cc) * P2K + (s - sd - 1))) * J.w2;
  int32_t* dst = ring + J.ring_in + ((int64_t)((d * 5 + cc) * RING + (s & RMASK))) * J.width;
  for (int c = threadIdx.x; c < J.width; c += blockDim.x) {
    const int k = c - J.koff;
    dst[c] = (k >= lo && k <= hi) ? src[k] : WF_NULL;
  }
}
void launch_p2_to_ring(int32_t* ring, const int32_t* p2, const P2Job* jobs, int njobs, hipStream_t st) {
  static_assert(P2K >= RING, "the snapshot after a round of phase 2 is taken from the P2 rows alone");
  hipLaunchKernelGGL(wfa_p2_to_ring_kernel, dim3((unsigned)njobs * 2 * 5 * RING), dim3(256), 0, st, ring, p2, jobs);
}
__global__ __launch_bounds__(256) void wfa_ring_widen_kernel(const RingWidenJob* __restrict__ jobs) {
  const RingWidenJob J = jobs[blockIdx.z];
  const int64_t c0 = ((int64_t)blockIdx.x * blockDim.x + threadIdx.x) * 4;
  if (c0 + 3 >= (int64_t)J.dst_w) return;
  const int64_t row = blockIdx.y;
  const int32_t* __restrict__ src = J.src + row * (int64_t)J.src_w;
  int32_t* __restrict__ dst = J.dst + row * (int64_t)J.dst_w;
  const int64_t delta = (int64_t)J.src_koff - J.dst_koff;
  const int64_t k0 = c0 - J.dst_koff, s0 = c0 + delta;
  int4 v = make_int4(WF_NULL, WF_NULL, WF_NULL, WF_NULL);
  const bool inside = k0 >= J.klo && k0 + 3 <= J.khi && s0 >= 0 && s0 + 3 < (int64_t)J.src_w;
  const bool aligned = ((delta & 3) == 0) && ((J.src_w & 3) == 0) && ((reinterpret_cast<uintptr_t>(J.src) & 15) == 0);
  if (inside && aligned) {
    v = *reinterpret_cast<const int4*>(src + s0);
  } else {
    int32_t e[4];
#pragma unroll
    for (int q = 0; q < 4; ++q) {
      const int64_t k = k0 + q, sc = s0 + q;
      e[q] = (k >= J.klo && k <= J.khi && sc >= 0 && sc < (int64_t)J.src_w) ? src[sc] : WF_NULL;
    }
    v = make_int4(e[0], e[1], e[2], e[3]);
  }
  if ((reinterpret_cast<uintptr_t>(J.dst) & 15) == 0) *reinterpret_cast<int4*>(dst + c0) = v;
  else { dst[c0] = v.x; dst[c0 + 1] = v.y; dst[c0 + 2] = v.z; dst[c0 + 3] = v.w; }
}
void launch_ring_widen(const RingWidenJob* jobs, int njobs, int max_dst_w, int ring_rows, hipStream_t st) {
  if (njobs <= 0 || max_dst_w <= 0) return;
  const unsigned chunks = (unsigned)((max_dst_w / 4 + 255) / 256);
  hipLaunchKernelGGL(wfa_ring_widen_kernel, dim3(chunks, (unsigned)(2 * 5 * ring_rows), (unsigned)njobs), dim3(256), 0, st, jobs);
}
void launch_p2_blockmax(const int32_t* ring, const int32_t* p2, const P2Job* jobs, int32_t* bmax, int32_t* p2max, int njobs, hipStream_t st) {
  hipLaunchKernelGGL(wfa_p2_blockmax_kernel, dim3(njobs * 2 * P2ROWS), dim3(256), 0, st, ring, p2, jobs, bmax, p2max);
}
void launch_p2_overlap(const int32_t* ring, const int32_t* p2, const P2Job* jobs, const int32_t* p2max, const int32_t* bmax,
                       BpResult* res, int njobs, int threads, int max_nblk, DevPen pen, int scope, hipStream_t st) {
  static const int count = getenv("WFM_P2_COUNT") ? atoi(getenv("WFM_P2_COUNT")) : 0;
  (void)max_nblk;
  static const int work_cap = getenv("WFM_P2_WORKCAP") ? std::max(1, std::min(P2WORK, atoi(getenv("WFM_P2_WORKCAP")))) : P2WORK;
  static const int cm_max = getenv("WFM_P2_COLMAX") ? std::max(0, std::min(P2CM, atoi(getenv("WFM_P2_COLMAX")))) : P2CM;
  hipLaunchKernelGGL(wfa_p2_overlap_kernel, dim3(njobs), dim3(threads), 0, st, ring, p2, jobs, p2max, bmax, res, pen, scope, count, work_cap, cm_max);
}
void launch_p2_exact(const int32_t* ring, const int32_t* p2, const P2Job* jobs, BpResult* res, int njobs, int threads, DevPen pen, int scope, hipStream_t st) {
  if (njobs <= 0) return;
  const char* e = getenv("WFM_P2_EXACT_REACH");
  const int reach = e ? std::max(1, atoi(e)) : P2TESTS;
  hipLaunchKernelGGL(wfa_p2_exact_kernel, dim3(njobs), dim3(std::max(64, std::min(1024, threads & ~63))), 0, st, ring, p2, jobs, res, pen, scope, reach);
}
void p2_counters(unsigned long long* out) { (void)hipMemcpyFromSymbol(out, HIP_SYMBOL(g_p2cnt), sizeof(unsigned long long) * 8); }
void launch_base(const uint8_t* seq, int32_t* a32, uint8_t* a8, uint32_t* rle, const BaseJob* jobs, BaseResult* res,
                 int njobs, DevPen pen, bool wide, int ring_rows, hipStream_t st) {
  if (ring_rows == RING) {
    if (wide) hipLaunchKernelGGL(r32::wfa_base_kernel<1024>, dim3(njobs), dim3(1024), 0, st, seq, a32, a8, rle, jobs, res, pen);
    else hipLaunchKernelGGL(r32::wfa_base_kernel<256>, dim3(njobs), dim3(256), 0, st, seq, a32, a8, rle, jobs, res, pen);
  } else {
    if (wide) hipLaunchKernelGGL(r128::wfa_base_kernel<1024>, dim3(njobs), dim3(1024), 0, st, seq, a32, a8, rle, jobs, res, pen);
    else hipLaunchKernelGGL(r128::wfa_base_kernel<256>, dim3(njobs), dim3(256), 0, st, seq, a32, a8, rle, jobs, res, pen);
  }
}
void launch_compact(const uint32_t* rle, const int64_t* off, const int64_t* cap, uint32_t* out, unsigned long long* total,
                    int64_t* out_start, int32_t* out_count, int nprob, hipStream_t st) {
  hipLaunchKernelGGL(rle_compact_kernel, dim3(nprob), dim3(256), 0, st, rle, off, cap, out, total, out_start, out_count);
}

}
```

wfmash_amd/csrc/wfa_plan.h:

```cpp
#ifndef WFM_WFA_PLAN_H_
#define WFM_WFA_PLAN_H_
#include <stddef.h>
#include <stdint.h>
#include <string.h>

#include <algorithm>
#include <climits>
#include <vector>

#include "../../include/wfmash_hip.h"
#include "wfa_rows.h"

namespace wfm {

struct Node {
  int32_t prob;
  int32_t pb, pl, tb, tl;
  int32_t cb, ce;
  int32_t score_rem;
  int32_t smax;
  int32_t endsfree;
  int32_t noband;
  int32_t sub;
  int32_t hinted;
// ... 130 lines not shown
  int L, R;
  rng_block(make_rng(pl, tl, sub), s0, s0 + T, L, R);
  return 2 * s0 > sub + 128 || R < L;
}
inline bool tile_job_beyond_limit(int pl, int tl, int sub, int limit, int s0, int T) {
  if (limit <= 0) return false;
  if (s0 >= limit) return true;
  int L, R;
  rng_block(make_rng(pl, tl, sub), s0, s0 + T, L, R);
  return 2 * s0 > sub + 128 || R < L;
}

inline bool fits_one_tile(int widest, int threads, int C) { return widest <= threads * C; }
inline int one_tile_threads(int widest, int threads, int C) { return std::min(threads, std::max(64, ((widest + C - 1) / C + 63) / 64 * 64)); }

inline void append_tile_tasks(TileChunkPlan& p, int job, int dir, int ntiles, int core, bool packed, int dirs = 3) {
  if (!((dirs >> dir) & 1)) return;
  std::vector<TileTask>& to = packed ? p.tasks : p.tasks_by;
  for (int t = 0; t < ntiles; ++t) to.push_back(TileTask{(int32_t)job, dir, t, core});
}
inline void close_task_list(TileChunkPlan& p) {
  p.n_pk = p.tasks.size();
  p.tasks.insert(p.tasks.end(), p.tasks_by.begin(), p.tasks_by.end());
}

inline void plan_tile_chunk(const TilePlanJob* jobs, size_t n, const TilePlanRules& r, TileChunkPlan& p, const uint8_t* dirs = nullptr) {
  const int chunk = r.chunk, T = r.T;
  auto block_range = [&](const TilePlanJob& j, int b, int& L, int& R) { rng_block(make_rng(j.pl, j.tl, j.sub), j.s0 + b * T, j.s0 + (b + 1) * T, L, R); };
  p.tasks.clear(); p.tasks_by.clear();
  p.core_c = r.core;
  p.threads_b.assign((size_t)chunk, r.threads);
  if (r.reg && r.C == 2) {
    std::vector<int> wb((size_t)chunk, 0);
    for (size_t i = 0; i < n; ++i) {
      if (!jobs[i].active) continue;
      int wmax = 0;
      for (int b = 0; b < chunk; ++b) {
        int L, R;
        block_range(jobs[i], b, L, R);
        wmax = std::max(wmax, R - L + 1);
        wb[(size_t)b] = std::max(wb[(size_t)b], wmax);
      }
    }
    if (fits_one_tile(wb[(size_t)chunk - 1], r.threads, r.C)) {
      for (int b = 0; b < chunk; ++b) {
        const int wdt = r.fine ? wb[(size_t)b] : wb[(size_t)chunk - 1];
        p.threads_b[(size_t)b] = r.fine ? one_tile_threads(wdt, r.threads, r.C) : std::min(r.threads, wdt <= 256 ? 128 : (wdt <= 512 ? 256 : r.threads));
      }
      p.core_c = p.threads_b[(size_t)chunk - 1] * r.C;
    }
  }
  for (size_t i = 0; i < n; ++i) {
    if (!jobs[i].active) continue;
    int ntiles = 0;
    for (int b = 0; b < chunk; ++b) {
      int L, R;
      block_range(jobs[i], b, L, R);
      ntiles = std::max(ntiles, tiles_for(L, R, p.core_c));
    }
    for (int d = 0; d < 2; ++d) append_tile_tasks(p, (int)i, d, ntiles, p.core_c, jobs[i].packed != 0, dirs ? dirs[i] : 3);
  }
  close_task_list(p);
  p.variants_b.assign((size_t)chunk, r.coarse_on ? 0 : 2);
  if (!r.coarse_on) return;
  for (size_t i = 0; i < n; ++i) {
    const TilePlanJob& j = jobs[i];
    if (!j.active || !(j.packed & 1)) continue;
    for (int b = 0; b < chunk; ++b) {
      const bool reaches = (int64_t)j.s0 + (int64_t)(b + 1) * T >= (int64_t)j.fine_s;
      if ((j.mode == 5 && b == 0) || (j.mode == 0 && reaches)) p.variants_b[(size_t)b] |= 2;
      if (j.mode == 0 && !reaches) p.variants_b[(size_t)b] |= 1;
    }
  }
  for (int b = 0; b < chunk; ++b) if (!p.variants_b[(size_t)b]) p.variants_b[(size_t)b] = r.planned ? 1 : 2;
}

inline int reuse_cadence(int every, int chunk) { return (std::max(1, every) + chunk - 1) / chunk * chunk; }
inline int reuse_resume_limit(int score_rem, int T, int fine_margin) {
  const int64_t x = (int64_t)score_rem / 2 - fine_margin;
  return x < 0 ? -1 : (int)(x / T * T - T);
}
inline int reuse_pick_keep(const int32_t* kept_s, size_t n, int score_rem, int T, int fine_margin, int min_blocks = 1) {
  if (score_rem == INT_MAX) return -1;
  const int limit = reuse_resume_limit(score_rem, T, fine_margin);
  const int64_t least = (int64_t)std::max(1, min_blocks) * T;
  int best = -1;
  for (size_t i = 0; i < n; ++i)
    if (kept_s[i] >= least && kept_s[i] <= limit && (best < 0 || kept_s[i] > kept_s[(size_t)best])) best = (int)i;
  return best;
}
inline bool reuse_ranges_contained(int ppl, int ptl, int psub, int cpl, int ctl, int csub, int s_k) {
  const Rng P = make_rng(ppl, ptl, psub), Cc = make_rng(cpl, ctl, csub);
  for (int s = std::max(0, s_k - RNG_BACK); s <= s_k; ++s) {
    const int lo = rng_lo(Cc, s), hi = rng_hi(Cc, s);
    if (hi < lo) continue;
    if (lo < rng_lo(P, s) || hi > rng_hi(P, s)) return false;
  }
  return true;
}
inline bool reuse_eligible(const Node& nd, const RingPlan& rp, int ppl, int ptl, int psub, int child_sub, int s_k, int T) {
  if (nd.keep <= 0 || nd.score_rem == INT_MAX || nd.sub == SUB_NONE || !rp.fits || !rp.tile_it || rp.band != 0 || rp.grown) return false;
  if (s_k < T || s_k % T != 0) return false;
  return reuse_ranges_contained(ppl, ptl, psub, nd.pl, nd.tl, child_sub, s_k);
}
inline bool reuse_keep_wanted(int es, int64_t s_meet, int cadence, int T) {
  if (s_meet <= 0) return false;
  return 100 * (int64_t)es >= 40 * s_meet - 100 * (64 + (int64_t)(2 + cadence) * T) && 100 * (int64_t)es <= 60 * s_meet;
}
inline int64_t reuse_meet_estimate(int s0, int64_t mak, int64_t A) { return s0 <= 0 || mak <= 0 ? 0 : (int64_t)s0 * A / mak; }
inline int reuse_keep_kmin(int pl, int s) { return std::max(-pl, -s); }
inline int reuse_keep_cols(int pl, int tl, int s) { return std::min(tl, s) - std::max(-pl, -s) + 1; }
inline size_t reuse_keep_elems(int pl, int tl, int s) { return (size_t)KEEP_ROWS * (size_t)reuse_keep_cols(pl, tl, s); }
struct ReuseKeeper { int pl, tl, upto; };
inline int reuse_fit_cadence(const ReuseKeeper* jobs, size_t n, int cadence, int T, size_t cap_bytes) {
  int upto_max = 0;
  for (size_t i = 0; i < n; ++i) upto_max = std::max(upto_max, jobs[i].upto);
  for (; (int64_t)cadence * T <= upto_max; cadence *= 2) {
    size_t bytes = 0;
    for (size_t i = 0; i < n && bytes <= cap_bytes; ++i)
      for (int64_t s = (int64_t)cadence * T; s <= jobs[i].upto && bytes <= cap_bytes; s += (int64_t)cadence * T) bytes += 2 * 4 * reuse_keep_elems(jobs[i].pl, jobs[i].tl, (int)s);
    if (bytes <= cap_bytes) return cadence;
  }
  return 0;
}

inline int planned_meet_sum(int score_rem, const wfm_penalties_t& pen, int comp_begin, int comp_end, bool second) {
  if (score_rem == INT_MAX || score_rem <= 0) return 0;
  const int cut = second ? comp_begin : comp_end;
  const int D = cut == 0 ? 0 : ((cut == 1 || cut == 3) ? pen.o1 : pen.o2);
  return std::max(0, score_rem - D);
}
struct PlannedMeet { int sf, sr, last_fwd; };
inline PlannedMeet planned_meet_state(int sum) { return PlannedMeet{(sum + 1) / 2, sum / 2, sum & 1}; }
inline PlannedMeet planned_meet(int score_rem, const wfm_penalties_t& pen, int comp_begin, int comp_end, bool second) {
  return planned_meet_state(planned_meet_sum(score_rem, pen, comp_begin, comp_end, second));
}
inline int planned_meet_block(int sum, int T) { return ((sum + 1) / 2 - 1) / T * T; }
inline bool planned_meet_eligible(const Node& nd, const RingPlan& rp, bool packed, int s_keep, int T) {
  if (nd.meet <= 0 || nd.score_rem == INT_MAX || nd.sub == SUB_NONE || !rp.fits || !rp.tile_it || rp.grown || !packed) return false;
  if (planned_meet_state(nd.meet).sf < 1) return false;
  return s_keep <= 0 || planned_meet_block(nd.meet, T) >= s_keep + T;
}

struct P2PlanJob { int pl, tl, sub, sf, sr, packed; };
struct P2Geometry {
  int koff2; size_t w2, nblk;
  size_t p2_off, bm_off;
};
struct P2ChunkPlan {
  std::vector<P2Geometry> geo;
  size_t elems = 0, bm_elems = 0, maxw2 = 0;
  int threads_c = 0;
  TileChunkPlan tiles;
};
inline void plan_p2_chunk(const P2PlanJob* cand, size_t n_cand, size_t i0, int rows, int rows_bm, size_t budget, int threads, int core, P2ChunkPlan& p,
                          const char* exact = nullptr) {
  p.geo.clear(); p.elems = 0; p.bm_elems = 0; p.maxw2 = 0;
  p.tiles.tasks.clear(); p.tiles.tasks_by.clear();
  for (size_t i = i0; i < n_cand; ++i) {
    const P2PlanJob& j = cand[i];
    const int reach = std::max(j.sf, j.sr) + rows;
    int L, R;
    rng_block(make_rng(j.pl, j.tl, j.sub), std::max(0, std::min(j.sf, j.sr) - P2_BACK), reach, L, R);
    if (R < L) { L = 0; R = 0; }
    P2Geometry g;
    g.koff2 = ((-L + 4) + 3) & ~3;
    g.w2 = ((size_t)(R + g.koff2 + 8) + 3) & ~(size_t)3;
    g.nblk = (g.w2 >> 6) + 1;
    const size_t need = g.w2 * 2 * 5 * rows, need_bm = (exact && exact[i]) ? 0 : g.nblk * 2 * rows_bm * 5;
    if (!p.geo.empty() && (p.elems + need + 2 * (p.bm_elems + need_bm)) * 4 > budget) break;
    p.maxw2 = std::max(p.maxw2, g.w2);
    g.p2_off = p.elems; g.bm_off = p.bm_elems;
    p.bm_elems += need_bm;
    p.elems += need;
    p.geo.push_back(g);
  }
  const size_t n = p.geo.size();
  auto dir_range = [&](const P2PlanJob& j, int d, int& L, int& R) { rng_block(make_rng(j.pl, j.tl, j.sub), d == 0 ? j.sf : j.sr, (d == 0 ? j.sf : j.sr) + rows, L, R); };
  p.threads_c = threads; p.tiles.core_c = core;
  int widest = 0;
  for (size_t q = 0; q < n; ++q)
    for (int d = 0; d < 2; ++d) {
      int L, R;
      dir_range(cand[i0 + q], d, L, R);
      widest = std::max(widest, R - L + 1);
    }
  if (fits_one_tile(widest, threads, 2)) {
    p.threads_c = one_tile_threads(widest, threads, 2);
    p.tiles.core_c = p.threads_c * 2;
  }
  for (size_t q = 0; q < n; ++q)
    for (int d = 0; d < 2; ++d) {
      int L, R;
      dir_range(cand[i0 + q], d, L, R);
      append_tile_tasks(p.tiles, (int)q, d, tiles_for(L, R, p.tiles.core_c), p.tiles.core_c, cand[i0 + q].packed != 0);
    }
  close_task_list(p.tiles);
}

inline int p2_exact_threads(size_t maxw2) {
  const size_t t = ((maxw2 + 3) / 4 + 63) / 64 * 64;
  return (int)std::min<size_t>(1024, std::max<size_t>(128, t));
}

inline void base_columns(const Node& nd, int pbf, int pef, int tbf, int tef, bool corner_band, int64_t* kmin_out, int64_t* kmax_out) {
  int64_t kmin = nd.endsfree ? std::max<int64_t>(-nd.pl, -(int64_t)pbf - nd.smax) : std::max<int64_t>(-nd.pl, -nd.smax);
  int64_t kmax = nd.endsfree ? std::min<int64_t>(nd.tl, (int64_t)tbf + nd.smax) : std::min<int64_t>(nd.tl, nd.smax);
  const bool end_fixed = !nd.endsfree || (pef == 0 && tef == 0);
  if (corner_band && end_fixed) {
    const int64_t k_end = (int64_t)nd.tl - nd.pl;
    const int64_t bmin = std::max(kmin, k_end - nd.smax), bmax = std::min(kmax, k_end + nd.smax);
    const int64_t lo0 = nd.endsfree ? std::max<int64_t>(-(int64_t)pbf, bmin) : 0, hi0 = nd.endsfree ? std::min<int64_t>((int64_t)tbf, bmax) : 0;
    if (bmin <= bmax && lo0 <= hi0 && lo0 >= bmin && hi0 <= bmax) { kmin = bmin; kmax = bmax; }
  }
  *kmin_out = kmin; *kmax_out = kmax;
}

struct BaseRules {
  bool base_v2 = true;
  bool base_tiles = true;
  bool force_tiles = false;
  bool few_jobs = false;
  int wide_from = 2048;
};
inline int base_kind(int64_t width, int pl, int tl, int tries, bool acgt, const BaseRules& r) {
  if (r.base_v2 && (pl == 0 || tl == 0)) return 1;
  if (r.base_v2 && width <= 2048 && acgt)
    return width <= 128 ? 0 : (r.base_tiles && (r.force_tiles || (r.few_jobs && (tries > 0 || width > 640))) ? 5 : (width <= 640 ? 1 : 2));
  if (r.base_v2 && r.base_tiles && acgt) return 5;
  return width > r.wide_from ? 4 : 3;
}

struct BaseTilePlan { int core = 0, nblocks = 0; std::vector<int> ntiles; };
inline BaseTilePlan plan_base_tiles(const int32_t* width, const int32_t* smax, size_t n, int T, int threads) {
  BaseTilePlan p;
  p.core = threads * 2 - 2 * T;
  p.ntiles.resize(n);
  int smax_all = 0;
  for (size_t q = 0; q < n; ++q) {
    p.ntiles[q] = (width[q] + p.core - 1) / p.core;
    smax_all = std::max(smax_all, smax[q]);
  }
  p.nblocks = (smax_all + T - 1) / T + 1;
  return p;
}

enum { EXPAND_OK = 0, EXPAND_SPANS = 1, EXPAND_ARENA = 2, EXPAND_RUN_TOO_LONG = 3 };
struct Expanded {
  int32_t score = -1;
  uint32_t n_runs = 0, ops_len = 0;
  uint64_t pc = 0, tc = 0;
};
inline int expand_runs(const uint32_t* e, int cnt, const wfm_penalties_t& pen, int plen, int tlen, char* ops, size_t ops_cap,
                       std::vector<uint32_t>* runs_out, Expanded* out) {
  static const char opc[4] = {'M', 'X', 'I', 'D'};
  const size_t runs_before = runs_out ? runs_out->size() : 0;
  int64_t score = 0;
  uint64_t pc = 0, tc = 0, both = 0;
  uint32_t nruns = 0;
  size_t pos = 0;
  int k = 0;
  while (k < cnt) {
    const int op = (int)(e[k] & 3u);
    uint64_t len = e[k] >> 2;
    int k2 = k + 1;
    while (k2 < cnt && (int)(e[k2] & 3u) == op) { len += e[k2] >> 2; ++k2; }
    if (runs_out) {
      if (len >= (1u << 30)) return EXPAND_RUN_TOO_LONG;
      runs_out->push_back((uint32_t)(len << 2) | (uint32_t)op);
    } else {
      if (pos + len > ops_cap) return EXPAND_ARENA;
      memset(ops + pos, opc[op], (size_t)len);
      pos += (size_t)len;
    }
    ++nruns;
    if (op == 1) { score += (int64_t)len * pen.x; pc += len; tc += len; both += len; }
    else if (op == 0) { pc += len; tc += len; both += len; }
    else {
      score += std::min<int64_t>(pen.o1 + (int64_t)len * pen.e1, pen.o2 + (int64_t)len * pen.e2);
      if (op == 2) tc += len; else pc += len;
    }
    k = k2;
  }
  out->pc = pc; out->tc = tc;
  if (pc != (uint64_t)plen || tc != (uint64_t)tlen) {
    if (runs_out) runs_out->resize(runs_before);
    return EXPAND_SPANS;
  }
  out->ops_len = runs_out ? (uint32_t)(pc + tc - both) : (uint32_t)pos;
  out->n_runs = nruns;
  out->score = (int32_t)score;
  return EXPAND_OK;
}

}
#endif
```

wfmash_amd/csrc/wfa_tile2.hip:

```cpp
#include <hip/hip_runtime.h>
#include <stdint.h>
#include <type_traits>

#include "wfa_device.h"
#include "wfa_base.h"
#include "wfa_pack.h"

#ifdef WFM_TILE_TRACE
__device__ unsigned long long g_tile_trace[48 * 16 * 128 * 4];
extern "C" int wfm_debug_tile_trace(unsigned long long* out, size_t n) {
  return (int)hipMemcpyFromSymbol(out, HIP_SYMBOL(g_tile_trace), n * sizeof(unsigned long long), 0, hipMemcpyDeviceToHost);
}
#if WFM_TILE_TRACE == 1
#define WFM_TRACE_STAMP(slot_) do { if (trace_on) { const unsigned long long ts_ = __builtin_readcyclecounter(); if (lane == 0) g_tile_trace[(((size_t)blockIdx.x * 16 + wv) * 128 + (t & 127)) * 4 + (slot_)] = ts_; } } while (0)
#else
#define WFM_TRACE_STAMP(slot_) do { } while (0)
#endif
#define WFM_TRACE_MARK(idx_) do { if (WFM_TILE_TRACE == 2 && trace_on2) { const unsigned long long ts_ = __builtin_readcyclecounter(); if (lane == 0) g_tile_trace[(((size_t)blockIdx.x * 16 + wv) * 128 + (idx_)) * 4] = ts_; } } while (0)
#else
#define WFM_TRACE_STAMP(slot_) do { } while (0)
#define WFM_TRACE_MARK(idx_) do { } while (0)
#endif

namespace wfm {
// ... 665 lines not shown
      fin[c] = pM[c] + pext[c];
      mak = max(mak, pM[c] >= 0 ? 2 * fin[c] + negk[c] : 0);
    }
    switch (Tn % UB) {
      case 1: line_take(std::integral_constant<int, 1>{}, fin); break;
      case 2: line_take(std::integral_constant<int, 2>{}, fin); break;
      case 3: line_take(std::integral_constant<int, 3>{}, fin); break;
      case 4: line_take(std::integral_constant<int, 4>{}, fin); break;
      case 5: line_take(std::integral_constant<int, 5>{}, fin); break;
      case 6: line_take(std::integral_constant<int, 6>{}, fin); break;
      case 7: line_take(std::integral_constant<int, 7>{}, fin); break;
      case 8: line_take(std::integral_constant<int, 8>{}, fin); break;
      case 9: line_take(std::integral_constant<int, 9>{}, fin); break;
      default: line_take(std::integral_constant<int, UB>{}, fin); break;
    }
    if (!FINE) (void)__hip_atomic_fetch_max(&s_run[tid], mak, __ATOMIC_RELAXED, __HIP_MEMORY_SCOPE_WORKGROUP);
    else slot_max(Tn - (Tn + UB - 1) / UB * UB, mak);
  }
  WFM_TRACE_MARK(122);
  if (P2) return;
  if (FAST) {
    const int r10 = Tn % UB;
#pragma unroll
    for (int j0 = 1; j0 <= NCL; ++j0) {
      if (r10 >= j0 && r10 < j0 + NCL) {
        const int clx = j0 % NCL;
#pragma unroll
        for (int c = 0; c < C; ++c) {
          const int parked = Mh[c][clx][DEP - 1];
#pragma unroll
          for (int e = DEP - 1; e > 0; --e) Mh[c][clx][e] = Mh[c][clx][e - 1];
          Mh[c][clx][0] = parked;
        }
      }
    }
  }
  const int s_end = s0 + Tn;
  if (Tn < H) {
#pragma unroll
    for (int c = 0; c < C; ++c) {
      const int k = k0 + c;
      if (!incore[c]) continue;
      for (int d = Tn; d < H; ++d) {
        const int sc = s_end - d;
        if (sc < 0 || k < rng_lo(RG, sc) || k > rng_hi(RG, sc)) continue;
        const int64_t ro = ((int64_t)(sc & RMASK)) * width + k;
        rout[(int64_t)C_I1 * RING * width + ro] = rin[(int64_t)C_I1 * RING * width + ro];
        rout[(int64_t)C_I2 * RING * width + ro] = rin[(int64_t)C_I2 * RING * width + ro];
        rout[(int64_t)C_D1 * RING * width + ro] = rin[(int64_t)C_D1 * RING * width + ro];
        rout[(int64_t)C_D2 * RING * width + ro] = rin[(int64_t)C_D2 * RING * width + ro];
      }
    }
  }
  const int k0w = __builtin_amdgcn_readfirstlane(k0);
  const bool lean_st = (coarse & 4) != 0 && tile_wave_lean_store(RG, k0w, tk.core_lo, tk.core_hi, s_end, Tn);
  int32_t* const wrow_out = rout + k0w;
  const unsigned lofs_out = (unsigned)lane * (unsigned)(C * sizeof(int32_t));
  auto write_rows = [&](auto TR) {
    constexpr int tr = decltype(TR)::value;
    if (lean_st) {
      if (incore[0])
#pragma unroll
      for (int d = 0; d < H; ++d) {
        const int r = ((tr - d) % NCL + NCL) % NCL, back = ((tr - r) % NCL + NCL) % NCL, e = (d - back) / NCL;
        char* const row = reinterpret_cast<char*>(wrow_out + ((int64_t)(C_M * RING + ((s_end - d) & RMASK))) * width);
        st_pair(reinterpret_cast<int32_t*>(row + lofs_out), Mh[0][r][e], Mh[1][r][e]);
      }
      return;
    }
    if (!incore[0] && !incore[1]) return;
#pragma unroll
    for (int d = 0; d < H; ++d) {
      constexpr int dummy = 0; (void)dummy;
      const int r = ((tr - d) % NCL + NCL) % NCL;
      const int back = ((tr - r) % NCL + NCL) % NCL;
      const int e = (d - back) / NCL;
      const int sc = s_end - d;
      const int lo = rng_lo(RG, sc), hi = rng_hi(RG, sc);
      const bool w0 = incore[0] && sc >= 0 && k0 >= lo && k0 <= hi, w1 = incore[1] && sc >= 0 && k0 + 1 >= lo && k0 + 1 <= hi;
      int32_t* dst = rout + ((int64_t)(C_M * RING + (sc & RMASK))) * width + k0;
      if (w0 && w1) st_pair(dst, Mh[0][r][e], Mh[1][r][e]);
      else {
        if (w0) dst[0] = Mh[0][r][e];
        if (w1) dst[1] = Mh[1][r][e];
      }
    }
  };
  switch (Tn % NCL) {
    case 0: write_rows(std::integral_constant<int, 0>{}); break;
    case 1: write_rows(std::integral_constant<int, 1>{}); break;
    case 2: write_rows(std::integral_constant<int, 2>{}); break;
    case 3: write_rows(std::integral_constant<int, 3>{}); break;
    default: write_rows(std::integral_constant<int, 4>{}); break;
  }
  int32_t* mk = mak_out + ((int64_t)tk.job * 2 + dir) * T;
  WFM_TRACE_MARK(123);
  if (!FINE) {
    if (J.mode == 0) {
      const int makrun = wave_max63(s_run[tid]);
      if (lane == 63 && makrun > 0) atomicMax(&mk[T - 1], makrun);
    }
    return;
  }
  __syncthreads();
  if (SLOTS) {
    for (int i0 = wv * 64; i0 < T * MS; i0 += NT) {
      const int i = i0 + lane;
      int v = i < T * MS ? s_makr[MS + i] : 0;
#pragma unroll
      for (int o = MS / 2; o > 0; o >>= 1) v = max(v, __shfl_xor(v, o));
      if ((i & (MS - 1)) == 0 && i < T * MS && v > 0) atomicMax(&mk[i / MS], v);
    }
    return;
  }
  for (int t = 1 + tid; t <= T; t += NT) if (s_makr[t] > 0) atomicMax(&mk[t - 1], s_makr[t]);
}

static bool tile_fast() {
  const char* e = getenv("WFM_TILE_FAST");
  return !(e && atoi(e) == 0);
}
static int tile_lean() {
  const char* e = getenv("WFM_TILE_LEAN");
  return (e && atoi(e) == 0) ? 0 : 4;
}
bool tile2_coarse_maxima() {
  const char* e = getenv("WFM_TILE_COARSE");
  return tile_fast() && !(e && atoi(e) == 0);
}
void launch_tile2(const uint32_t* pk, int32_t* ring, const TileJob* jobs, const TileTask* tasks, int32_t* mak, int ntasks, int threads, int T,
                  int variants, hipStream_t st) {
  const size_t lds1 = (size_t)(T + 1) * 4;
  const int lean = tile_lean();
  if (tile_fast()) {
    const int coarse = tile2_coarse_maxima() ? 1 : 0;
    if (!coarse) variants = 2;
    const size_t pad = getenv("WFM_TILE_LDS_PAD") ? (size_t)atoi(getenv("WFM_TILE_LDS_PAD")) : 0;
    if (variants & 1) {
      if (threads <= 64) hipLaunchKernelGGL((wfa_tile2_kernel<64, false, true, false>), dim3(ntasks), dim3(64), 0, st, pk, ring, jobs, tasks, mak, T, (int32_t*)nullptr, coarse | lean);
      else hipLaunchKernelGGL((wfa_tile2_kernel<1024, false, true, false>), dim3(ntasks), dim3(threads), pad, st, pk, ring, jobs, tasks, mak, T, (int32_t*)nullptr, coarse | lean);
    }
    if (variants & 2) {
      const int cf = coarse | (variants == 2 ? 2 : 0);
      const size_t ldsm = lds1 * (size_t)tile_fine_slots(threads);
      if (threads <= 64) hipLaunchKernelGGL((wfa_tile2_kernel<64, false, true, true, TILE_SLOTS_WAVE1>), dim3(ntasks), dim3(64), ldsm, st, pk, ring, jobs, tasks, mak, T, (int32_t*)nullptr, cf | lean);
      else if (threads <= 128) hipLaunchKernelGGL((wfa_tile2_kernel<1024, false, true, true, TILE_SLOTS_SMALL>), dim3(ntasks), dim3(threads), ldsm, st, pk, ring, jobs, tasks, mak, T, (int32_t*)nullptr, cf | lean);
      else hipLaunchKernelGGL((wfa_tile2_kernel<1024, false, true, true, TILE_SLOTS_WIDE>), dim3(ntasks), dim3(threads), ldsm, st, pk, ring, jobs, tasks, mak, T, (int32_t*)nullptr, cf | lean);
    }
  } else {
    if (threads <= 64) hipLaunchKernelGGL((wfa_tile2_kernel<64, false, false, true>), dim3(ntasks), dim3(64), lds1, st, pk, ring, jobs, tasks, mak, T, (int32_t*)nullptr, lean);
    else hipLaunchKernelGGL((wfa_tile2_kernel<1024, false, false, true>), dim3(ntasks), dim3(threads), lds1, st, pk, ring, jobs, tasks, mak, T, (int32_t*)nullptr, lean);
  }
}
void launch_tile2_p2(const uint32_t* pk, int32_t* ring, const TileJob* jobs, const TileTask* tasks, int ntasks, int threads, int32_t* p2, hipStream_t st) {
  const size_t lds1 = (size_t)(P2K + 1) * 4;
  const int lean = tile_lean();
  if (tile_fast()) {
    if (threads <= 64) hipLaunchKernelGGL((wfa_tile2_kernel<64, true, true, false>), dim3(ntasks), dim3(64), 0, st, pk, ring, jobs, tasks, (int32_t*)nullptr, P2K, p2, lean);
    else hipLaunchKernelGGL((wfa_tile2_kernel<1024, true, true, false>), dim3(ntasks), dim3(threads), 0, st, pk, ring, jobs, tasks, (int32_t*)nullptr, P2K, p2, lean);
  } else {
    if (threads <= 64) hipLaunchKernelGGL((wfa_tile2_kernel<64, true, false, true>), dim3(ntasks), dim3(64), lds1, st, pk, ring, jobs, tasks, (int32_t*)nullptr, P2K, p2, lean);
    else hipLaunchKernelGGL((wfa_tile2_kernel<1024, true, false, true>), dim3(ntasks), dim3(threads), lds1, st, pk, ring, jobs, tasks, (int32_t*)nullptr, P2K, p2, lean);
  }
}

constexpr int B2_C = 2, B2_NCL = 5, B2_DEP = 6, B2_E1 = 2;
constexpr DevPen B2_PEN{5, 8, 2, 24, 1};

__device__ __forceinline__ PkSrc b2_load_windows(const BaseJob& J, const uint32_t* __restrict__ pk, uint32_t* s_winP, uint32_t* s_winT, int tid, int stride,
                                                 int& dP, int& dT) {
  const int64_t oriP = J.p_off & ~(int64_t)15, oriT = J.t_off & ~(int64_t)15;
  dP = (int)(J.p_off - oriP); dT = (int)(J.t_off - oriT);
  PkSrc SRC;
  SRC.lP = (lds_words)s_winP; SRC.lT = (lds_words)s_winT;
  SRC.gP = (glb_words)pk + (oriP >> 4); SRC.gT = (glb_words)pk + (oriT >> 4);
  const int nP = min(PK_WIN_DW + PK_SLACK_DW, (J.pl + dP + 15) / 16 + 8), nT = min(PK_WIN_DW + PK_SLACK_DW, (J.tl + dT + 15) / 16 + 8);
  for (int i = tid; i < nP; i += stride) s_winP[i] = SRC.gP[i];
  for (int i = tid; i < nT; i += stride) s_winT[i] = SRC.gT[i];
  return SRC;
}

__device__ __forceinline__ void b2_end_checks(const BaseJob& J, int* s_done, int* s_endk, int k, int m_ext, int ins1, int ins2, int del1, int del2) {
  const int pl = J.pl, tl = J.tl;
  if (J.endsfree) {
    if (m_ext >= 0) {
      const int h = m_ext, v = m_ext - k;
      if ((h >= tl && pl - v <= J.pef) || (v >= pl && tl - h <= J.tef)) atomicMin(s_endk, k);
    }
  } else if (k == tl - pl) {
    const int ev = J.comp_end == C_M ? m_ext : (J.comp_end == C_I1 ? ins1 : (J.comp_end == C_I2 ? ins2 : (J.comp_end == C_D1 ? del1 : del2)));
    if (ev >= tl) *s_done = 1;
  }
}

__device__ __forceinline__ void b2_row0(const BaseJob& J, const PkSrc& SRC, int dT, int lo0, int hi0, int k0, const int (&cP)[B2_C], const bool (&keep)[B2_C],
                                        int32_t* pre_base, uint8_t* bt_base, int* s_done, int* s_endk, int (&Mh)[B2_C][B2_NCL][B2_DEP], int (&I1h)[B2_C][B2_E1],
                                        int (&D1h)[B2_C][B2_E1], int (&I2h)[B2_C], int (&D2h)[B2_C], int (&mcur)[B2_C]) {
  constexpr int C = B2_C;
  const int pl = J.pl, tl = J.tl, k_end = tl - pl;
  int m0[C], ext[C], maxn[C];
  unsigned oP[C], oT[C];
#pragma unroll
  for (int c = 0; c < C; ++c) {
    const int k = k0 + c;
    const bool on = k >= lo0 && k <= hi0;
    int m = WF_NULL;
    if (on) {
      if (J.endsfree) m = k > 0 ? k : 0;
      else {
        if (J.comp_begin == C_M) m = 0;
        I1h[c][0] = J.comp_begin == C_I1 ? 0 : WF_NULL;
        I2h[c] = J.comp_begin == C_I2 ? 0 : WF_NULL;
        D1h[c][0] = J.comp_begin == C_D1 ? 0 : WF_NULL;
        D2h[c] = J.comp_begin == C_D2 ? 0 : WF_NULL;
      }
    }
    m0[c] = m;
    oP[c] = (unsigned)(m + cP[c]); oT[c] = (unsigned)(m + dT);
    maxn[c] = m >= 0 ? min(pl - (m - k), tl - m) : 0;
  }
  pk_extend2(SRC, m0, oP, oT, maxn, ext);
#pragma unroll
  for (int c = 0; c < C; ++c) {
    const int k = k0 + c;
    if (k < lo0 || k > hi0) continue;
    if (keep[c]) { pre_base[k] = m0[c]; bt_base[k] = 0; }
    int m = m0[c];
    if (m >= 0) m += ext[c];
    if (keep[c]) {
      if (J.endsfree) b2_end_checks(J, s_done, s_endk, k, m, WF_NULL, WF_NULL, WF_NULL, WF_NULL);
      else if (k == k_end && J.comp_end == C_M && m >= tl) *s_done = 1;
    }
    Mh[c][0][0] = m;
    mcur[c] = m;
  }
}

template <bool WAVE1, int NWV>
__device__ __forceinline__ void b2_publish_edges(int (&s_edge)[2][NWV][2][4], int par, int wv, int lane, int cl, const int (&Mh)[B2_C][B2_NCL][B2_DEP],
                                                 const int (&I1h)[B2_C][B2_E1], const int (&D1h)[B2_C][B2_E1], const int (&I2h)[B2_C], const int (&D2h)[B2_C]) {
  constexpr int C = B2_C, E1 = B2_E1;
  if (WAVE1) return;
  if (lane == 63) { int* e = s_edge[par][wv][0]; e[0] = Mh[C - 1][cl][1]; e[1] = Mh[C - 1][cl][4]; e[2] = I1h[C - 1][E1 - 1]; e[3] = I2h[C - 1]; }
  if (lane == 0)  { int* e = s_edge[par][wv][1]; e[0] = Mh[0][cl][1];     e[1] = Mh[0][cl][4];     e[2] = D1h[0][E1 - 1];     e[3] = D2h[0]; }
}
template <bool WAVE1, int NWV>
__device__ __forceinline__ void b2_neighbours(const int (&s_edge)[2][NWV][2][4], int par, int wv, int nw, int lane, int cl,
                                              const int (&Mh)[B2_C][B2_NCL][B2_DEP], const int (&I1h)[B2_C][B2_E1], const int (&D1h)[B2_C][B2_E1],
                                              const int (&I2h)[B2_C], const int (&D2h)[B2_C], int& lM10, int& lM25, int& lI1, int& lI2, int& rM10, int& rM25,
                                              int& rD1, int& rD2) {
  constexpr int C = B2_C, E1 = B2_E1;
  lM10 = from_prev_lane(Mh[C - 1][cl][1]); lM25 = from_prev_lane(Mh[C - 1][cl][4]);
  lI1 = from_prev_lane(I1h[C - 1][E1 - 1]); lI2 = from_prev_lane(I2h[C - 1]);
  rM10 = from_next_lane(Mh[0][cl][1]); rM25 = from_next_lane(Mh[0][cl][4]);
  rD1 = from_next_lane(D1h[0][E1 - 1]); rD2 = from_next_lane(D2h[0]);
  if (WAVE1) return;
  if (lane == 0 && wv > 0) { const int* e = s_edge[par][wv - 1][0]; lM10 = e[0]; lM25 = e[1]; lI1 = e[2]; lI2 = e[3]; }
  if (lane == 63 && wv + 1 < nw) { const int* e = s_edge[par][wv + 1][1]; rM10 = e[0]; rM25 = e[1]; rD1 = e[2]; rD2 = e[3]; }
}

__device__ __forceinline__ void b2_cells(const int (&Mh)[B2_C][B2_NCL][B2_DEP], const int (&I1h)[B2_C][B2_E1], const int (&D1h)[B2_C][B2_E1], const int (&I2h)[B2_C],
                                         const int (&D2h)[B2_C], int cl, int lM10, int lM25, int lI1, int lI2, int rM10, int rM25, int rD1, int rD2,
                                         const unsigned (&hmaxu)[B2_C], const bool (&colok)[B2_C], int k0, int lo, int hi, int (&nM)[B2_C], int (&nI1)[B2_C],
                                         int (&nI2)[B2_C], int (&nD1)[B2_C], int (&nD2)[B2_C], unsigned (&btb)[B2_C]) {
  constexpr int C = B2_C, E1 = B2_E1;
#pragma unroll
  for (int c = 0; c < C; ++c) {
    const int k = k0 + c;
    const int a10 = c == 0 ? lM10 : Mh[c - 1][cl][1], b10 = c == C - 1 ? rM10 : Mh[c + 1][cl][1];
    const int a25 = c == 0 ? lM25 : Mh[c - 1][cl][4], b25 = c == C - 1 ? rM25 : Mh[c + 1][cl][4];
    const int i1 = c == 0 ? lI1 : I1h[c - 1][E1 - 1], d1 = c == C - 1 ? rD1 : D1h[c + 1][E1 - 1];
    const int i2 = c == 0 ? lI2 : I2h[c - 1], d2 = c == C - 1 ? rD2 : D2h[c + 1];
    const int mx = Mh[c][cl][0];
    unsigned bits = 0;
    if (i1 >= a10) bits |= BT_I1_EXT;
    if (i2 >= a25) bits |= BT_I2_EXT;
    if (d1 >= b10) bits |= BT_D1_EXT;
    if (d2 >= b25) bits |= BT_D2_EXT;
    const unsigned hm = hmaxu[c];
    int ins1 = max(a10, i1) + 1, ins2 = max(a25, i2) + 1, del1 = max(b10, d1), del2 = max(b25, d2), mis = mx + 1;
    ins1 = (unsigned)ins1 <= hm ? ins1 : WF_NULL;
    ins2 = (unsigned)ins2 <= hm ? ins2 : WF_NULL;
    del1 = (unsigned)del1 <= hm ? del1 : WF_NULL;
    del2 = (unsigned)del2 <= hm ? del2 : WF_NULL;
    mis = (unsigned)mis <= hm ? mis : WF_NULL;
    int m = ins1; unsigned src = C_I1;
    if (ins2 >= m) { m = ins2; src = C_I2; }
    if (del1 >= m) { m = del1; src = C_D1; }
    if (del2 >= m) { m = del2; src = C_D2; }
    if (mis >= m)  { m = mis;  src = C_M; }
    const bool on = k >= lo && k <= hi;
    nI1[c] = on ? ins1 : WF_NULL; nI2[c] = on ? ins2 : WF_NULL; nD1[c] = on ? del1 : WF_NULL; nD2[c] = on ? del2 : WF_NULL;
    nM[c] = (on && colok[c]) ? m : WF_NULL;
    btb[c] = bits | src;
  }
}
__device__ __forceinline__ void b2_shift(int (&Mh)[B2_C][B2_NCL][B2_DEP], int (&I1h)[B2_C][B2_E1], int (&D1h)[B2_C][B2_E1], int (&I2h)[B2_C], int (&D2h)[B2_C],
                                         int (&mcur)[B2_C], int cl, const int (&nM)[B2_C], const int (&nI1)[B2_C], const int (&nI2)[B2_C],
                                         const int (&nD1)[B2_C], const int (&nD2)[B2_C]) {
#pragma unroll
  for (int c = 0; c < B2_C; ++c) {
    mcur[c] = nM[c];
#pragma unroll
    for (int e = B2_DEP - 1; e > 0; --e) Mh[c][cl][e] = Mh[c][cl][e - 1];
    Mh[c][cl][0] = nM[c];
#pragma unroll
    for (int d = B2_E1 - 1; d > 0; --d) { I1h[c][d] = I1h[c][d - 1]; D1h[c][d] = D1h[c][d - 1]; }
    I1h[c][0] = nI1[c]; D1h[c][0] = nD1[c];
    I2h[c] = nI2[c]; D2h[c] = nD2[c];
  }
}

__device__ __forceinline__ int& b2_snap_reg(int (&M)[B2_NCL][B2_DEP], int (&I1)[B2_E1], int (&D1)[B2_E1], int& I2, int& D2, int row) {
  static_assert(B2T_ROWS == SNAP_ROWS + 2 * B2_E1 + 2, "the snapshot's rows");
  if (row < SNAP_ROWS) return M[(B2_NCL - row % B2_NCL) % B2_NCL][row / B2_NCL];
// ... 389 lines not shown
```

wfmash_amd/host/capi_host.cpp:

```cpp
#include <algorithm>
#include <exception>
#include <iostream>
#include <string>
#include <thread>
#include <vector>

#include "../../include/wfmash_host.h"
#include "../csrc/wfa_handle.h"
#include "../csrc/wfa_pack.h"
#include "../csrc/wfa_plan.h"
#include "../csrc/wfa_optband.h"
#include "aligner.hpp"
#include "fasta.hpp"
#include "chain_text.hpp"
#include "lift_text.hpp"
#include "transitive_text.hpp"
#include "pav_text.hpp"
#include "genotype_text.hpp"
#include "map_stats.hpp"

extern "C" {

int wfmh_test_packed_lce(const uint8_t* buf_p, int64_t n_p, int64_t start_p, const uint8_t* buf_t, int64_t n_t, int64_t start_t, int v, int h, int maxn) {
  if (!buf_p || !buf_t || n_p < 0 || n_t < 0 || start_p < 0 || start_t < 0 || v < 0 || h < 0) return -1;
// ... 361 lines not shown
    switch (q[0]) {
      case 0: out[0] = wfm::cells_sum(q[1], q[2], q[3], q[4], q[5]); break;
      case 1: wfm::rng_block(wfm::make_rng(q[1], q[2], q[3]), q[4], q[5], a, b); out[0] = a; out[1] = b; break;
      case 2: wfm::tile_span(q[1], q[2], q[3], q[4], &a, &b); out[0] = a; out[1] = b; break;
      case 3: out[0] = wfm::tiles_for(q[1], q[2], q[3]); break;
      case 4: case 5: out[0] = wfm::tile_job_leaves(q[1], q[2], q[3], q[4], q[5], q[6], q[0] == 4 ? 100 : 32); break;
      case 6: case 7: out[0] = wfm::tile_job_beyond_limit(q[1], q[2], q[3], q[4], q[5], q[0] == 6 ? 100 : 32); break;
      default: return -1;
    }
  }
  return 0;
}

int wfmh_test_tile_interior(const int32_t* q, int64_t n, int32_t* out) {
  for (int64_t i = 0; i < n; ++i, q += 7, out += 3) {
    const wfm::Rng r = wfm::make_rng(q[0], q[1], q[2]);
    out[0] = wfm::rng_interior(r, q[3], q[4], q[5], q[6]) ? 1 : 0;
    out[1] = wfm::rng_lo(r, q[5]);
    out[2] = wfm::rng_hi(r, q[5]);
  }
  return 0;
}

int wfmh_test_tile_lean_waves(const int32_t* in, int64_t* out) {
  const wfm::Rng r = wfm::make_rng(in[0], in[1], in[2]);
  const int s0 = in[3], T = in[4], Tn = in[5], core = in[6], threads = in[7];
  if (T < 1 || core < 1 || threads < 64) return -1;
  int L, R;
  wfm::rng_block(r, s0, s0 + T, L, R);
  const int nt = wfm::tiles_for(L, R, core);
  out[0] = nt; out[1] = out[2] = out[3] = out[4] = 0;
  for (int idx = 0; idx < nt; ++idx) {
    int lo, hi;
    wfm::tile_span(L, R, idx, core, &lo, &hi);
    const int halo = (lo == L && hi == R) ? 0 : T;
    const int kA = lo - halo, kmax = hi + halo;
    const int nw = std::min(threads / 64, (kmax - kA) / wfm::WAVE_DIAGS + 1);
    int lean_here = 0;
    for (int w = 0; w < nw; ++w) {
      const int kw = kA + w * wfm::WAVE_DIAGS;
      out[1] += 1;
      lean_here += wfm::tile_wave_lean_load(r, kw, kmax, s0) ? 1 : 0;
      out[3] += wfm::tile_wave_lean_store(r, kw, lo, hi, s0 + Tn, Tn) ? 1 : 0;
    }
    out[2] += lean_here;
    out[4] += (lean_here > 0 && lean_here < nw) ? 1 : 0;
  }
  return 0;
}

int wfmh_test_opt_band(const int64_t* in, int64_t* out) {
  if (!in || !out || in[5] < 0 || in[6] < 0 || in[11] < 0) return -1;
  const wfm::OptBand b = wfm::opt_band(wfm::OptPen{in[0], in[1], in[2], in[3], in[4]}, in[5], in[6], in[7], in[8], in[9], in[10], in[11]);
  out[0] = b.lo; out[1] = b.hi; out[2] = (int64_t)b.cells;
  return 0;
}

int wfmh_test_tile_plan(const int32_t* jobs, int64_t n, const int32_t* rules, int32_t* per_block, int32_t* tasks, int64_t tasks_cap, int64_t* scalars) {
  static_assert(sizeof(wfm::TilePlanJob) == 8 * sizeof(int32_t) && sizeof(wfm::TileTask) == 4 * sizeof(int32_t), "the hooks copy these as rows of int32");
  wfm::TilePlanRules r{rules[0], rules[1], rules[2], rules[3], rules[4], rules[5] != 0, rules[6] != 0, rules[7] != 0};
  if (r.chunk < 1 || r.T < 1 || r.threads < 1 || r.C < 1 || r.core < 1) return -1;
  wfm::TileChunkPlan p;
  wfm::plan_tile_chunk(reinterpret_cast<const wfm::TilePlanJob*>(jobs), (size_t)n, r, p);
  std::copy(p.threads_b.begin(), p.threads_b.end(), per_block);
  std::copy(p.variants_b.begin(), p.variants_b.end(), per_block + r.chunk);
  memcpy(tasks, p.tasks.data(), std::min<size_t>(p.tasks.size(), (size_t)tasks_cap) * sizeof(wfm::TileTask));
  scalars[0] = p.core_c; scalars[1] = (int64_t)p.tasks.size(); scalars[2] = (int64_t)p.n_pk;
  return 0;
}

int wfmh_test_reuse_plan(int op, const int64_t* in, int64_t n, int64_t* out) {
  if (op == 0) {
    std::vector<int32_t> kept((size_t)n);
    for (int64_t i = 0; i < n; ++i) kept[(size_t)i] = (int32_t)in[4 + i];
    out[0] = wfm::reuse_pick_keep(kept.data(), kept.size(), (int)in[0], (int)in[1], (int)in[2], (int)in[3]);
    out[1] = in[0] == INT_MAX ? -1 : wfm::reuse_resume_limit((int)in[0], (int)in[1], (int)in[2]);
    return 0;
  }
  if (op == 1) {
    wfm::Node nd{};
    nd.pl = (int32_t)in[0]; nd.tl = (int32_t)in[1]; nd.score_rem = (int32_t)in[2]; nd.keep = (int32_t)in[4];
    nd.sub = nd.score_rem == INT_MAX ? wfm::SUB_NONE : nd.score_rem + 56;
    wfm::RingPlan rp;
    rp.fits = in[5] != 0; rp.tile_it = in[6] != 0; rp.band = (int)in[7]; rp.grown = in[8] != 0;
    out[0] = wfm::reuse_eligible(nd, rp, (int)in[9], (int)in[10], (int)in[11], (int)in[3], (int)in[12], (int)in[13]);
    return 0;
  }
  if (op == 2) {
    if (in[0] < 1 || in[1] < 1 || in[2] < 1) return -1;
    std::vector<wfm::ReuseKeeper> kp((size_t)n);
    for (int64_t i = 0; i < n; ++i) kp[(size_t)i] = wfm::ReuseKeeper{(int)in[4 + 3 * i], (int)in[5 + 3 * i], (int)in[6 + 3 * i]};
    out[0] = wfm::reuse_cadence((int)in[0], (int)in[1]);
    out[1] = wfm::reuse_fit_cadence(kp.data(), kp.size(), (int)out[0], (int)in[2], (size_t)in[3]);
    return 0;
  }
  if (op == 3) {
    out[1] = wfm::reuse_meet_estimate((int)in[0], in[2], in[3]);
    out[0] = wfm::reuse_keep_wanted((int)in[1], out[1], (int)in[4], (int)in[5]);
    return 0;
  }
  return -1;
}

int wfmh_test_planned_meet(const int64_t* in, int64_t n, int64_t* out) {
  for (int64_t i = 0; i < n; ++i, in += 16, out += 8) {
    wfm_penalties_t pen{};
    pen.x = (int)in[0]; pen.o1 = (int)in[1]; pen.e1 = (int)in[2]; pen.o2 = (int)in[3]; pen.e2 = (int)in[4];
    const int T = (int)in[15];
    if (T < 1) return -1;
    const int sum = wfm::planned_meet_sum((int)in[5], pen, (int)in[6], (int)in[7], in[8] != 0);
    const wfm::PlannedMeet m = wfm::planned_meet((int)in[5], pen, (int)in[6], (int)in[7], in[8] != 0);
    const int b0 = wfm::planned_meet_block(sum, T);
    wfm::Node nd{};
    nd.score_rem = (int32_t)in[5]; nd.cb = (int32_t)in[6]; nd.ce = (int32_t)in[7]; nd.sub = (int32_t)in[9]; nd.meet = sum;
    wfm::RingPlan rp;
    rp.fits = in[10] != 0; rp.tile_it = in[11] != 0; rp.grown = in[12] != 0;
    out[0] = sum; out[1] = m.sf; out[2] = m.sr; out[3] = m.last_fwd; out[4] = b0; out[5] = m.sf - b0; out[6] = m.sr - b0;
    out[7] = wfm::planned_meet_eligible(nd, rp, in[13] != 0, (int)in[14], T) ? 1 : 0;
  }
  return 0;
}

int wfmh_test_tile_plan_dirs(const int32_t* jobs, int64_t n, const int32_t* rules, const uint8_t* dirs, int32_t* per_block, int32_t* tasks, int64_t tasks_cap,
                             int64_t* scalars) {
  wfm::TilePlanRules r{rules[0], rules[1], rules[2], rules[3], rules[4], rules[5] != 0, rules[6] != 0, rules[7] != 0};
  if (r.chunk < 1 || r.T < 1 || r.threads < 1 || r.C < 1 || r.core < 1) return -1;
  wfm::TileChunkPlan p;
  wfm::plan_tile_chunk(reinterpret_cast<const wfm::TilePlanJob*>(jobs), (size_t)n, r, p, dirs);
  std::copy(p.threads_b.begin(), p.threads_b.end(), per_block);
  std::copy(p.variants_b.begin(), p.variants_b.end(), per_block + r.chunk);
  memcpy(tasks, p.tasks.data(), std::min<size_t>(p.tasks.size(), (size_t)tasks_cap) * sizeof(wfm::TileTask));
  scalars[0] = p.core_c; scalars[1] = (int64_t)p.tasks.size(); scalars[2] = (int64_t)p.n_pk;
  return 0;
}

int wfmh_test_p2_plan(const int32_t* cand, int64_t n, int64_t i0, int rows, int rows_bm, unsigned long long budget, int threads, int core, int64_t* geo,
                      int32_t* tasks, int64_t tasks_cap, int64_t* scalars) {
  static_assert(sizeof(wfm::P2PlanJob) == 6 * sizeof(int32_t), "the hook copies these as rows of int32");
  if (i0 < 0 || i0 >= n || rows < 1 || threads < 1 || core < 1) return -1;
  wfm::P2ChunkPlan p;
  wfm::plan_p2_chunk(reinterpret_cast<const wfm::P2PlanJob*>(cand), (size_t)n, (size_t)i0, rows, rows_bm, (size_t)budget, threads, core, p);
  for (size_t q = 0; q < p.geo.size(); ++q) {
    const wfm::P2Geometry& g = p.geo[q];
    const int64_t v[5] = {g.koff2, (int64_t)g.w2, (int64_t)g.nblk, (int64_t)g.p2_off, (int64_t)g.bm_off};
    std::copy(v, v + 5, geo + 5 * q);
  }
  memcpy(tasks, p.tiles.tasks.data(), std::min<size_t>(p.tiles.tasks.size(), (size_t)tasks_cap) * sizeof(wfm::TileTask));
  const int64_t v[8] = {(int64_t)p.geo.size(), (int64_t)p.elems, (int64_t)p.bm_elems, (int64_t)p.maxw2, p.threads_c, p.tiles.core_c,
                        (int64_t)p.tiles.tasks.size(), (int64_t)p.tiles.n_pk};
  std::copy(v, v + 8, scalars);
  return 0;
}

int wfmh_test_base_plan(int op, const int32_t* in, int64_t n, int32_t* out) {
  if (op == 0) {
    for (int64_t i = 0; i < n; ++i, in += 10)
      out[i] = wfm::base_kind(in[0], in[1], in[2], in[3], in[4] != 0, wfm::BaseRules{in[5] != 0, in[6] != 0, in[7] != 0, in[8] != 0, in[9]});
    return 0;
  }
  if (op != 1 || in[0] < 1 || in[1] * 2 <= 2 * in[0]) return -1;
  std::vector<int32_t> width((size_t)n), smax((size_t)n);
  for (int64_t i = 0; i < n; ++i) { width[(size_t)i] = in[2 + 2 * i]; smax[(size_t)i] = in[3 + 2 * i]; }
  const wfm::BaseTilePlan p = wfm::plan_base_tiles(width.data(), smax.data(), (size_t)n, in[0], in[1]);
  out[0] = p.core; out[1] = p.nblocks;
  std::copy(p.ntiles.begin(), p.ntiles.end(), out + 2);
  return 0;
}

char* wfmh_test_cigar(const char* fn, const char* a, const char* b, const char* query, const char* target,
                      long long i0, long long i1) {
  std::string f = fn ? fn : "", sa = a ? a : "", sb = b ? b : "", q = query ? query : "", t = target ? target : "";
  std::string r;
  const wflign::CigarOps o2 = wflign::parse_cigar(sb);
  wflign::CigarOps o = wflign::parse_cigar(sa);
  auto erosion = [](const wflign::Erosion& e, size_t third) { return std::to_string(e.query_eroded) + "," + std::to_string(e.target_eroded) + "," + std::to_string(third); };
  if (f == "erode") { wflign::erode_short_matches_in_cigar(o, (int)i0, i1 != 0); r = wflign::cigar_to_string(o); }
  else if (f == "merge") { wflign::merge_adjacent_ops(o, o2, 0, o2.size()); r = wflign::cigar_to_string(o); }
  else if (f == "compress") r = wflign::compress_ops(sa.data(), sa.size());
  else if (f == "swap_start") { wflign::try_swap_start_pattern(o, q.data(), (int64_t)q.size(), t.data(), (int64_t)t.size()); r = wflign::cigar_to_string(o); }
  else if (f == "swap_end") { wflign::try_swap_end_pattern(o, q.data(), (int64_t)q.size(), t.data(), (int64_t)t.size()); r = wflign::cigar_to_string(o); }
  else if (f == "head_erosion") {
    const wflign::Erosion e = wflign::scan_head_erosion(o);
    r = erosion(e, wflign::cigar_to_string(o, 0, e.erode_end_pos).size());
  } else if (f == "tail_erosion") {
    const wflign::Erosion e = wflign::scan_tail_erosion(o);
    r = erosion(e, e.erode_start_idx);
  } else if (f == "patch_plan") {
    const wflign::PatchPlan pl = wflign::plan_patches(o);
    r = erosion(pl.head, pl.head.erode_end_pos) + "," + erosion(pl.tail, pl.tail.erode_start_idx) + "," + std::to_string((int)pl.head_wanted) + "," +
        std::to_string((int)pl.tail_wanted) + "," + std::to_string((int)pl.tail_independent);
  } else if (f == "runs") {
    std::vector<uint32_t> runs;
    std::stringstream ss(sa);
    std::string item;
    while (std::getline(ss, item, ',')) if (!item.empty()) runs.push_back((uint32_t)std::stoul(item));
    wflign::ops_from_runs(runs.data(), runs.size(), o);
    r = wflign::cigar_to_string(o);
  } else if (f == "paf") {
    std::vector<std::string> p;
    std::stringstream ss(sb);
    std::string item;
    while (std::getline(ss, item, '|')) p.push_back(item);
    if (p.size() == 12) {
      wflign::PafParams pp;
      wflign::write_alignment_paf(r, o, p[0], std::stoull(p[1]), std::stoull(p[2]), std::stoull(p[3]), p[4] == "1", p[5],
                                  std::stoull(p[6]), std::stoull(p[7]), pp, std::stof(p[8]), std::stoi(p[9]), std::stoi(p[10]),
                                  std::stoi(p[11]));
    }
  } else if (f == "min_hits") {
    int sk = 0, k = 0; float id = 0, ci = 0;
    if (sscanf(sa.c_str(), "%d,%d,%f,%f", &sk, &k, &id, &ci) == 4)
      r = std::to_string(skch::Stat::estimateMinimumHits(sk, k, id)) + "," + std::to_string(skch::Stat::estimateMinimumHitsRelaxed(sk, k, id, ci));
  } else if (f == "sketch_cutoffs") {
    int sk = 0, k = 0; float ad = 0, ac = 0;
    if (sscanf(sa.c_str(), "%d,%d,%f,%f", &sk, &k, &ad, &ac) == 4)
      for (int v : skch::Stat::sketch_cutoffs(sk, k, ad, ac)) { if (!r.empty()) r += ","; r += std::to_string(v); }
  } else if (f == "l2_tables") {
    int S = 0, k = 0; float id = 0, ci = 0;
    if (sscanf(sa.c_str(), "%d,%d,%f,%f", &S, &k, &id, &ci) == 4) {
      std::vector<uint8_t> keep;
      std::vector<uint16_t> ident;
      skch::Stat::l2_identity_tables(S, k, id, true, ci, keep, ident);
      for (size_t i = 0; i < keep.size(); ++i) { if (i) r += ","; r += std::to_string((int)keep[i]) + ":" + std::to_string((int)ident[i]); }
    }
  } else if (f == "md") {
    r = wflign::md_string(o, 0, o.size(), (int)i0, t.c_str());
  } else if (f == "parse_row") {
    try {
      align::MappingBoundaryRow row;
      align::Aligner::parseMashmapRow(sa, row, (uint64_t)i0, (uint64_t)i1);
      std::ostringstream os;
      os << row.qId << "," << row.qStartPos << "," << row.qEndPos << "," << (row.strand == align::FWD ? "+" : "-") << ","
         << row.refId << "," << row.rStartPos << "," << row.rEndPos << "," << row.mashmap_estimated_identity << ","
         << row.chain_id << "," << row.chain_length << "," << row.chain_pos;
      r = os.str();
    } catch (const std::exception& e) { r = std::string("ERROR"); }
  }
  char* out = (char*)malloc(r.size() + 1);
  memcpy(out, r.c_str(), r.size() + 1);
  return out;
}

char* wfmh_test_fasta(const char* path, const char* name, int64_t start, int64_t end_inclusive, int whole) {
  std::string r;
  try {
    wfmash_host::FastaStore fa(path ? path : "");
    if (!name) {
      std::ostringstream os;
      os << (fa.indexed() ? "indexed" : "in-memory") << "\n";
      for (int i = 0; i < fa.nseq(); ++i) os << fa.name(i) << "\t" << fa.length(i) << "\n";
      r = os.str();
    } else {
      const int i = fa.find(name);
      if (i < 0) r = "ERROR: no such sequence";
      else {
        if (whole) fa.preload({i}, std::max(2, whole));
        r = fa.fetch(name, start, end_inclusive);
      }
    }
  } catch (const std::exception& e) {
    r = std::string("ERROR: ") + e.what();
  }
  char* out = (char*)malloc(r.size() + 1);
  if (!out) return nullptr;
  memcpy(out, r.data(), r.size());
  out[r.size()] = 0;
  return out;
}

}

void wfmh_release_sequences(void) { wfmash_host::release_kept(); }

char* wfmh_test_fasta_shared(const char* path, const char* name) {
  std::string r;
  try {
    std::shared_ptr<wfmash_host::FastaStore> fa = wfmash_host::open_shared(path ? path : "");
    const int i = name ? fa->find(name) : -1;
    if (i < 0) r = "ERROR: no such sequence";
    else { const wfmash_host::SeqView v = fa->sequence(i, 1); r.assign(v.data(), v.size()); }
    wfmash_host::keep_until_next({fa});
  } catch (const std::exception& e) {
    r = std::string("ERROR: ") + e.what();
  }
  char* out = (char*)malloc(r.size() + 1);
  if (!out) return nullptr;
  memcpy(out, r.data(), r.size());
  out[r.size()] = 0;
  return out;
}
```

Before: 69.39 million aligned bases/s.

## Compute fewer phase-2 rows ahead for jobs expected to take the exact walk

Phase-2 planning now splits jobs into search jobs and exact-walk jobs. Exact-walk jobs get a shorter row count derived from the gap-open penalties, (max(o1,o2)+2)/2, and their own tile plan and launch. When the exact walk misses with reduced rows, the full P2K rows are recomputed for those jobs before the search kernel runs. This removes wavefront row computation that the exact walk does not need, at the cost of an extra launch set and recompute on misses.

```diff
diff --git a/include/wfmash_host.h b/include/wfmash_host.h
--- a/include/wfmash_host.h
+++ b/include/wfmash_host.h
@@ -121,6 +121,8 @@
 int wfmh_test_tile_plan(const int32_t* jobs, int64_t n, const int32_t* rules, int32_t* per_block, int32_t* tasks, int64_t tasks_cap, int64_t* scalars);
 int wfmh_test_p2_plan(const int32_t* cand, int64_t n, int64_t i0, int rows, int rows_bm, unsigned long long budget, int threads, int core, int64_t* geo,
                       int32_t* tasks, int64_t tasks_cap, int64_t* scalars);
+int wfmh_test_p2_plan_kinds(const int32_t* cand, int64_t n, int64_t i0, int rows, int rows_bm, unsigned long long budget, int threads, int core,
+                            const char* exact, int rows_exact, const int32_t* pen_o, int32_t* tasks, int64_t tasks_cap, int64_t* scalars);
 int wfmh_test_base_plan(int op, const int32_t* in, int64_t n, int32_t* out);
 int wfmh_test_reuse_plan(int op, const int64_t* in, int64_t n, int64_t* out);
 int wfmh_test_planned_meet(const int64_t* in, int64_t n, int64_t* out);
diff --git a/wfmash_amd/capi.py b/wfmash_amd/capi.py
--- a/wfmash_amd/capi.py
+++ b/wfmash_amd/capi.py
@@ -1742,7 +1742,7 @@
                 "wfmh_map_default_params", "wfmh_test_filter", "wfmh_map", "wfmh_test_winnow_chunked", "wfmh_test_fasta", "wfmh_test_winnow_thinned", "wfmh_test_sort_records", "wfmh_test_index_file",
                 "wfmh_map_multi", "wfmh_align_paf_multi", "wfmh_test_winnow_model", "wfmh_test_sortlike_model", "wfmh_test_finish_records",
                 "wfmh_release_sequences", "wfmh_test_fasta_shared", "wfmh_seed_paf", "wfmh_test_deal", "wfmh_test_subwindow",
-                "wfmh_test_rows", "wfmh_test_tile_plan", "wfmh_test_p2_plan", "wfmh_test_base_plan", "wfmh_test_map_plan", "wfmh_test_filter_ordered",
+                "wfmh_test_rows", "wfmh_test_tile_plan", "wfmh_test_p2_plan", "wfmh_test_p2_plan_kinds", "wfmh_test_base_plan", "wfmh_test_map_plan", "wfmh_test_filter_ordered",
                 "wfmh_test_reuse_plan", "wfmh_test_planned_meet", "wfmh_test_tile_plan_dirs", "wfmh_test_tile_interior", "wfmh_test_tile_lean_waves", "wfmh_set_verify", "wfmh_verify_counts", "wfmh_verify_paf", "wfmh_test_verify_parse",
                 "wfmh_set_verify_optimal", "wfmh_verify_optimal_counts", "wfmh_test_opt_band", "wfmh_set_left_align", "wfmh_left_align_counts", "wfmh_set_cs", "wfmh_cs_counts", "wfmh_set_variants", "wfmh_variants_counts",
                 "wfmh_set_coverage", "wfmh_coverage_counts", "wfmh_coverage_paf", "wfmh_test_coverage_bedgraph",
diff --git a/wfmash_amd/csrc/wfa_device.h b/wfmash_amd/csrc/wfa_device.h
--- a/wfmash_amd/csrc/wfa_device.h
+++ b/wfmash_amd/csrc/wfa_device.h
@@ -405,7 +405,7 @@
 constexpr int TILE_SLOTS_WAVE1 = 2, TILE_SLOTS_SMALL = 4, TILE_SLOTS_WIDE = WFM_TILE_SLOTS_WIDE;
 constexpr int tile_fine_slots(int threads) { return threads <= 64 ? TILE_SLOTS_WAVE1 : (threads <= 128 ? TILE_SLOTS_SMALL : TILE_SLOTS_WIDE); }
 bool tile2_coarse_maxima();
-void launch_tile2_p2(const uint32_t* pk, int32_t* ring, const TileJob* jobs, const TileTask* tasks, int ntasks, int threads, int32_t* p2, hipStream_t st);
+void launch_tile2_p2(const uint32_t* pk, int32_t* ring, const TileJob* jobs, const TileTask* tasks, int ntasks, int threads, int rows, int32_t* p2, hipStream_t st);
 int selftest_dpp(int* host_out128, hipStream_t st);
 void launch_base2(const uint32_t* pk, int32_t* a32, uint8_t* a8, uint32_t* rle, const BaseJob* jobs, BaseResult* res, int njobs, int threads, hipStream_t st);
 void launch_bp(const uint8_t* seq, int32_t* ring, const BpJob* jobs, BpResult* res, int njobs, int threads,
@@ -416,7 +416,7 @@
 void launch_tile_advance(TileJob* jobs, int32_t* mak, int njobs, int T, DevPen pen, int exact, int coarse, int launched, hipStream_t st);
 void launch_tile_reg(const uint8_t* seq, int32_t* ring, const TileJob* jobs, const TileTask* tasks, int32_t* mak, int ntasks,
                      int threads, int T, int C, bool cut, hipStream_t st);
-void launch_tile_p2(const uint8_t* seq, int32_t* ring, const TileJob* jobs, const TileTask* tasks, int ntasks, int threads,
+void launch_tile_p2(const uint8_t* seq, int32_t* ring, const TileJob* jobs, const TileTask* tasks, int ntasks, int threads, int rows,
                     int32_t* p2, bool cut, hipStream_t st);
 void launch_p2_to_ring(int32_t* ring, const int32_t* p2, const P2Job* jobs, int njobs, hipStream_t st);
 struct RingWidenJob {
@@ -430,7 +430,7 @@
 void launch_p2_blockmax(const int32_t* ring, const int32_t* p2, const P2Job* jobs, int32_t* bmax, int32_t* p2max, int njobs, hipStream_t st);
 void launch_p2_overlap(const int32_t* ring, const int32_t* p2, const P2Job* jobs, const int32_t* p2max, const int32_t* bmax,
                        BpResult* res, int njobs, int threads, int max_nblk, DevPen pen, int scope, hipStream_t st);
-void launch_p2_exact(const int32_t* ring, const int32_t* p2, const P2Job* jobs, BpResult* res, int njobs, int threads, DevPen pen, int scope, hipStream_t st);
+void launch_p2_exact(const int32_t* ring, const int32_t* p2, const P2Job* jobs, BpResult* res, int njobs, int threads, int rows, DevPen pen, int scope, hipStream_t st);
 void launch_base(const uint8_t* seq, int32_t* a32, uint8_t* a8, uint32_t* rle, const BaseJob* jobs, BaseResult* res,
                  int njobs, DevPen pen, bool wide, int ring_rows, hipStream_t st);
 void launch_compact(const uint32_t* rle, const int64_t* off, const int64_t* cap, uint32_t* out, unsigned long long* total,
diff --git a/wfmash_amd/csrc/wfa_host.hip b/wfmash_amd/csrc/wfa_host.hip
--- a/wfmash_amd/csrc/wfa_host.hip
+++ b/wfmash_amd/csrc/wfa_host.hip
@@ -890,13 +890,21 @@
   std::vector<int> at;
   std::vector<P2Job> pj_dev;
   size_t ns = 0, ns_dump = 0;
+  int rows_x = P2K;
+  size_t n_again = 0;
   std::vector<BpResult> got;
   float ms = 0;
 };
 
+int p2_rows_exact(const DevPen& dp) {
+  const char* e = getenv("WFM_P2_EXACT_ROWS");
+  const int r = e ? atoi(e) : p2_exact_rows(dp);
+  return r <= 0 ? P2K : std::min(r, P2K);
+}
+
 void fill_p2_chunk(P2Chunk& c, size_t i0) {
   const size_t budget = std::max<size_t>(c.h->mem_budget / 4, (size_t)64 << 20);
-  plan_p2_chunk(c.pcand.data(), c.pcand.size(), i0, P2K, P2ROWS, budget, c.cfg.threads, c.cfg.Wt - 2 * P2K, c.plan, c.pexact.data());
+  plan_p2_chunk(c.pcand.data(), c.pcand.size(), i0, P2K, P2ROWS, budget, c.cfg.threads, c.cfg.Wt - 2 * P2K, c.plan, c.pexact.data(), c.rows_x);
   c.i0 = i0; c.n = c.plan.geo.size();
   c.tj.clear(); c.pj.clear();
   c.at.assign(c.n, 0); c.ns = 0;
@@ -922,21 +930,27 @@
 int launch_p2_chunk(P2Chunk& c) {
   wfm_handle* h = c.h;
   wfm_seqset* S = c.S;
-  const size_t n = c.n, ns = c.ns, elems = c.plan.elems, bm_elems = c.plan.bm_elems, n_pk = c.plan.tiles.n_pk;
+  const size_t n = c.n, ns = c.ns, elems = c.plan.elems, bm_elems = c.plan.bm_elems;
   const std::vector<TileTask>& tasks = c.plan.tiles.tasks;
-  const int threads_c = c.plan.threads_c;
+  const std::vector<TileTask>& tasks_x = c.plan.tiles_x.tasks;
   if (h->p2rows.ensure(elems + 16) || h->p2max.ensure(ns * 2 * P2ROWS * 5) || h->p2bmax.ensure(bm_elems + 16) ||
-      h->p2jobs.ensure(n) || h->tilejobs.ensure(n) || h->tiletasks.ensure(tasks.size()) || h->bpres.ensure(std::max(n, c.jobs.size()))) {
+      h->p2jobs.ensure(n) || h->tilejobs.ensure(n) || h->tiletasks.ensure(tasks.size() + tasks_x.size()) || h->bpres.ensure(std::max(n, c.jobs.size()))) {
     h->err = "out of device memory (phase-2 rows)"; return WFM_E_NOMEM;
   }
   HIPCHK(h, hipMemcpyAsync(h->tilejobs.p, c.tj.data(), n * sizeof(TileJob), hipMemcpyHostToDevice, h->stream));
   HIPCHK(h, hipMemcpyAsync(h->p2jobs.p, c.pj_dev.data(), n * sizeof(P2Job), hipMemcpyHostToDevice, h->stream));
-  HIPCHK(h, hipMemcpyAsync(h->tiletasks.p, tasks.data(), tasks.size() * sizeof(TileTask), hipMemcpyHostToDevice, h->stream));
+  if (!tasks.empty()) HIPCHK(h, hipMemcpyAsync(h->tiletasks.p, tasks.data(), tasks.size() * sizeof(TileTask), hipMemcpyHostToDevice, h->stream));
+  if (!tasks_x.empty()) HIPCHK(h, hipMemcpyAsync(h->tiletasks.p + tasks.size(), tasks_x.data(), tasks_x.size() * sizeof(TileTask), hipMemcpyHostToDevice, h->stream));
   HIPCHK(h, hipEventRecord(h->ev0, h->stream));
   bool any_cut = false;
   for (const TileJob& t : c.tj) any_cut |= t.sub != SUB_NONE;
-  if (n_pk) launch_tile2_p2(S->d_pk, h->ring.p, h->tilejobs.p, h->tiletasks.p, (int)n_pk, threads_c, h->p2rows.p, h->stream);
-  if (tasks.size() > n_pk) launch_tile_p2(S->d_seq, h->ring.p, h->tilejobs.p, h->tiletasks.p + n_pk, (int)(tasks.size() - n_pk), threads_c, h->p2rows.p, any_cut, h->stream);
+  auto launch_rows = [&](const TileChunkPlan& t, size_t at, int threads_c, int rows) {
+    const size_t n_pk = t.n_pk;
+    if (n_pk) launch_tile2_p2(S->d_pk, h->ring.p, h->tilejobs.p, h->tiletasks.p + at, (int)n_pk, threads_c, rows, h->p2rows.p, h->stream);
+    if (t.tasks.size() > n_pk) launch_tile_p2(S->d_seq, h->ring.p, h->tilejobs.p, h->tiletasks.p + at + n_pk, (int)(t.tasks.size() - n_pk), threads_c, rows, h->p2rows.p, any_cut, h->stream);
+  };
+  launch_rows(c.plan.tiles, 0, c.plan.threads_c, P2K);
+  launch_rows(c.plan.tiles_x, tasks.size(), c.plan.threads_x, c.plan.rows_x);
   static const int p2_threads = getenv("WFM_P2_THREADS") ? atoi(getenv("WFM_P2_THREADS")) : 0;
   static const int p2x_threads = getenv("WFM_P2_EXACT_THREADS") ? atoi(getenv("WFM_P2_EXACT_THREADS")) : 0;
   auto launch_search = [&](size_t cnt) {
@@ -945,7 +959,7 @@
                       p2_threads > 0 ? p2_threads : 1024, (int)(c.plan.maxw2 >> 6) + 1, c.dp, c.scope, h->stream);
   };
   if (ns) launch_search(ns);
-  launch_p2_exact(h->ring.p, h->p2rows.p, h->p2jobs.p + ns, h->bpres.p + ns, (int)(n - ns), p2x_threads > 0 ? p2x_threads : p2_exact_threads(c.plan.maxw2), c.dp, c.scope, h->stream);
+  launch_p2_exact(h->ring.p, h->p2rows.p, h->p2jobs.p + ns, h->bpres.p + ns, (int)(n - ns), p2x_threads > 0 ? p2x_threads : p2_exact_threads(c.plan.maxw2), c.plan.rows_x, c.dp, c.scope, h->stream);
   HIPCHK(h, hipGetLastError());
   HIPCHK(h, hipEventRecord(h->ev1, h->stream));
   std::vector<BpResult> dev(n);
@@ -965,6 +979,7 @@
   c.ns_dump = ns;
   h->tile_ctr[WFM_TC_P2_EXACT] += n - ns;
   std::vector<size_t> miss;
+  c.n_again = 0;
   for (size_t q = 0; q < n; ++q) if (c.got[q].status == WFM_DEV_P2_EXACT_MISS) miss.push_back(q);
   if (!miss.empty()) {
     h->tile_ctr[WFM_TC_P2_EXACT_MISSES] += miss.size();
@@ -978,7 +993,17 @@
     }
     if (h->p2max.ensure(mj.size() * 2 * P2ROWS * 5) || h->p2bmax.ensure(bm + 16)) { h->err = "out of device memory (phase-2 maxima)"; return WFM_E_NOMEM; }
     HIPCHK(h, hipMemcpyAsync(h->p2jobs.p, mj.data(), mj.size() * sizeof(P2Job), hipMemcpyHostToDevice, h->stream));
+    TileChunkPlan tiles_m;
+    int threads_m = 0;
+    if (c.plan.rows_x < P2K) {
+      std::vector<int> which(miss.begin(), miss.end());
+      plan_p2_tiles(c.pcand.data(), c.i0, which, P2K, c.cfg.threads, c.cfg.Wt - 2 * P2K, tiles_m, threads_m);
+      if (h->tiletasks.ensure(tiles_m.tasks.size())) { h->err = "out of device memory (phase-2 rows)"; return WFM_E_NOMEM; }
+      HIPCHK(h, hipMemcpyAsync(h->tiletasks.p, tiles_m.tasks.data(), tiles_m.tasks.size() * sizeof(TileTask), hipMemcpyHostToDevice, h->stream));
+      c.n_again = miss.size();
+    }
     HIPCHK(h, hipEventRecord(h->ev0, h->stream));
+    if (!tiles_m.tasks.empty()) launch_rows(tiles_m, 0, threads_m, P2K);
     launch_search(mj.size());
     HIPCHK(h, hipGetLastError());
     HIPCHK(h, hipEventRecord(h->ev1, h->stream));
@@ -1027,9 +1052,9 @@
   size_t missed = 0;
   for (size_t q = 0; q < n; ++q) missed += pj[q].exact == 0 && (size_t)c.at[q] >= c.ns;
   fprintf(stderr, "[wfm] phase 2 from rows computed ahead: %zu jobs, widest %zu columns, %zu tiles of %d threads, %.3f ms, %d left to the step kernel; walk per job: %.1f rounds (max %d), %.0f us (max %.0f), of which cells stage %.0f us; "
-          "%.1f tests (max %d); exact walk %.1f %% of the jobs, missed %.1f %%\n",
+          "%.1f tests (max %d); exact walk %.1f %% of the jobs, missed %.1f %%; rows ahead %d, of the exact jobs %d in %zu tiles of %d threads, computed again for %zu\n",
           n, c.plan.maxw2, c.plan.tiles.tasks.size(), c.plan.threads_c, c.ms, more, rd / n, rdmax, tk / n / 100.0, tkmax / 100.0, tc / n / 100.0, tests / n, tests_max,
-          100.0 * (n - c.ns) / n, 100.0 * missed / n);
+          100.0 * (n - c.ns) / n, 100.0 * missed / n, P2K, c.plan.rows_x, c.plan.tiles_x.tasks.size(), c.plan.threads_x, c.n_again);
   size_t qs = 0;
   for (size_t q = 0; q < n; ++q) if (got[q].ticks_p2 > got[qs].ticks_p2) qs = q;
   fprintf(stderr, "[wfm]   slowest walk: pl %d tl %d sub %d w2 %d nblk %d: %d rounds, %.0f us = listing %.0f + cells %.0f (incl. listing) + pick %.0f, %u blocks listed, status %d\n", pj[qs].pl, pj[qs].tl,
@@ -1070,6 +1095,7 @@
                  std::vector<BpResult>& carry, std::vector<char>& has_carry, bool may_continue, std::vector<int>& again, const std::vector<int32_t>& exact_of) {
   if (cand.empty()) return WFM_OK;
   P2Chunk c{h, S, dp, scope, cfg, jobs, cand, ring_other, res, ms_out, carry, has_carry, may_continue, again, exact_of};
+  c.rows_x = p2_rows_exact(dp);
   for (size_t i = 0; i < cand.size(); ++i) {
     const BpJob& j = jobs[(size_t)cand[i]];
     c.pcand.push_back(P2PlanJob{j.pl, j.tl, j.sub, j.resume_s, j.resume_sr, j.packed});
diff --git a/wfmash_amd/csrc/wfa_kernels.hip b/wfmash_amd/csrc/wfa_kernels.hip
--- a/wfmash_amd/csrc/wfa_kernels.hip
+++ b/wfmash_amd/csrc/wfa_kernels.hip
@@ -1447,13 +1447,13 @@
   else if (cut) hipLaunchKernelGGL((wfa_tile_reg_kernel<2, 1024, 5, 10, 25, 2, 1, false, true>), dim3(ntasks), dim3(threads), lds, st, seq, ring, jobs, tasks, mak, T);
   else hipLaunchKernelGGL((wfa_tile_reg_kernel<2, 1024, 5, 10, 25, 2, 1, false, false>), dim3(ntasks), dim3(threads), lds, st, seq, ring, jobs, tasks, mak, T);
 }
-void launch_tile_p2(const uint8_t* seq, int32_t* ring, const TileJob* jobs, const TileTask* tasks, int ntasks, int threads,
+void launch_tile_p2(const uint8_t* seq, int32_t* ring, const TileJob* jobs, const TileTask* tasks, int ntasks, int threads, int rows,
                     int32_t* p2, bool cut, hipStream_t st) {
-  const size_t lds = (size_t)(P2K + 1) * 4;
+  const size_t lds = (size_t)(rows + 1) * 4;
   if (cut) hipLaunchKernelGGL((wfa_tile_reg_kernel<2, 1024, 5, 10, 25, 2, 1, true, true>), dim3(ntasks), dim3(threads), lds, st, seq, ring, jobs, tasks,
-                              (int32_t*)nullptr, P2K, p2, (int32_t*)nullptr);
+                              (int32_t*)nullptr, rows, p2, (int32_t*)nullptr);
   else hipLaunchKernelGGL((wfa_tile_reg_kernel<2, 1024, 5, 10, 25, 2, 1, true, false>), dim3(ntasks), dim3(threads), lds, st, seq, ring, jobs, tasks,
-                          (int32_t*)nullptr, P2K, p2, (int32_t*)nullptr);
+                          (int32_t*)nullptr, rows, p2, (int32_t*)nullptr);
 }
 __global__ __launch_bounds__(256) void wfa_p2_to_ring_kernel(int32_t* __restrict__ ring, const int32_t* __restrict__ p2, const P2Job* __restrict__ jobs) {
   const int job = blockIdx.x / (2 * 5 * RING), rest = blockIdx.x % (2 * 5 * RING), d = rest / (5 * RING), cc = (rest / RING) % 5, r = rest % RING;
@@ -1514,10 +1514,10 @@
   static const int cm_max = getenv("WFM_P2_COLMAX") ? std::max(0, std::min(P2CM, atoi(getenv("WFM_P2_COLMAX")))) : P2CM;
   hipLaunchKernelGGL(wfa_p2_overlap_kernel, dim3(njobs), dim3(threads), 0, st, ring, p2, jobs, p2max, bmax, res, pen, scope, count, work_cap, cm_max);
 }
-void launch_p2_exact(const int32_t* ring, const int32_t* p2, const P2Job* jobs, BpResult* res, int njobs, int threads, DevPen pen, int scope, hipStream_t st) {
+void launch_p2_exact(const int32_t* ring, const int32_t* p2, const P2Job* jobs, BpResult* res, int njobs, int threads, int rows, DevPen pen, int scope, hipStream_t st) {
   if (njobs <= 0) return;
   const char* e = getenv("WFM_P2_EXACT_REACH");
-  const int reach = e ? std::max(1, atoi(e)) : P2TESTS;
+  const int reach = std::min(2 * rows, e ? std::max(1, atoi(e)) : P2TESTS);
   hipLaunchKernelGGL(wfa_p2_exact_kernel, dim3(njobs), dim3(std::max(64, std::min(1024, threads & ~63))), 0, st, ring, p2, jobs, res, pen, scope, reach);
 }
 void p2_counters(unsigned long long* out) { (void)hipMemcpyFromSymbol(out, HIP_SYMBOL(g_p2cnt), sizeof(unsigned long long) * 8); }
diff --git a/wfmash_amd/csrc/wfa_plan.h b/wfmash_amd/csrc/wfa_plan.h
--- a/wfmash_amd/csrc/wfa_plan.h
+++ b/wfmash_amd/csrc/wfa_plan.h
@@ -306,11 +306,38 @@
   size_t elems = 0, bm_elems = 0, maxw2 = 0;
   int threads_c = 0;
   TileChunkPlan tiles;
-};
+  int rows_x = 0, threads_x = 0;
+  TileChunkPlan tiles_x;
+};
+template <class Pen>
+inline int p2_exact_rows(const Pen& pen) { return (std::max(pen.o1, pen.o2) + 2) / 2; }
+inline void plan_p2_tiles(const P2PlanJob* cand, size_t i0, const std::vector<int>& which, int rows, int threads, int core, TileChunkPlan& t, int& threads_c) {
+  t.tasks.clear(); t.tasks_by.clear();
+  auto dir_range = [&](const P2PlanJob& j, int d, int& L, int& R) { rng_block(make_rng(j.pl, j.tl, j.sub), d == 0 ? j.sf : j.sr, (d == 0 ? j.sf : j.sr) + rows, L, R); };
+  threads_c = threads; t.core_c = core;
+  int widest = 0;
+  for (int q : which)
+    for (int d = 0; d < 2; ++d) {
+      int L, R;
+      dir_range(cand[i0 + (size_t)q], d, L, R);
+      widest = std::max(widest, R - L + 1);
+    }
+  if (fits_one_tile(widest, threads, 2)) {
+    threads_c = one_tile_threads(widest, threads, 2);
+    t.core_c = threads_c * 2;
+  }
+  for (int q : which)
+    for (int d = 0; d < 2; ++d) {
+      int L, R;
+      dir_range(cand[i0 + (size_t)q], d, L, R);
+      append_tile_tasks(t, q, d, tiles_for(L, R, t.core_c), t.core_c, cand[i0 + (size_t)q].packed != 0);
+    }
+  close_task_list(t);
+}
 inline void plan_p2_chunk(const P2PlanJob* cand, size_t n_cand, size_t i0, int rows, int rows_bm, size_t budget, int threads, int core, P2ChunkPlan& p,
-                          const char* exact = nullptr) {
+                          const char* exact = nullptr, int rows_exact = 0) {
   p.geo.clear(); p.elems = 0; p.bm_elems = 0; p.maxw2 = 0;
-  p.tiles.tasks.clear(); p.tiles.tasks_by.clear();
+  p.tiles_x.tasks.clear(); p.tiles_x.tasks_by.clear(); p.tiles_x.n_pk = 0; p.tiles_x.core_c = 0; p.threads_x = 0;
   for (size_t i = i0; i < n_cand; ++i) {
     const P2PlanJob& j = cand[i];
     const int reach = std::max(j.sf, j.sr) + rows;
@@ -330,26 +357,11 @@
     p.geo.push_back(g);
   }
   const size_t n = p.geo.size();
-  auto dir_range = [&](const P2PlanJob& j, int d, int& L, int& R) { rng_block(make_rng(j.pl, j.tl, j.sub), d == 0 ? j.sf : j.sr, (d == 0 ? j.sf : j.sr) + rows, L, R); };
-  p.threads_c = threads; p.tiles.core_c = core;
-  int widest = 0;
-  for (size_t q = 0; q < n; ++q)
-    for (int d = 0; d < 2; ++d) {
-      int L, R;
-      dir_range(cand[i0 + q], d, L, R);
-      widest = std::max(widest, R - L + 1);
-    }
-  if (fits_one_tile(widest, threads, 2)) {
-    p.threads_c = one_tile_threads(widest, threads, 2);
-    p.tiles.core_c = p.threads_c * 2;
-  }
-  for (size_t q = 0; q < n; ++q)
-    for (int d = 0; d < 2; ++d) {
-      int L, R;
-      dir_range(cand[i0 + q], d, L, R);
-      append_tile_tasks(p.tiles, (int)q, d, tiles_for(L, R, p.tiles.core_c), p.tiles.core_c, cand[i0 + q].packed != 0);
-    }
-  close_task_list(p.tiles);
+  p.rows_x = (exact && rows_exact > 0 && rows_exact < rows) ? rows_exact : rows;
+  std::vector<int> search, walk;
+  for (size_t q = 0; q < n; ++q) (p.rows_x < rows && exact[i0 + q] ? walk : search).push_back((int)q);
+  plan_p2_tiles(cand, i0, search, rows, threads, core, p.tiles, p.threads_c);
+  if (!walk.empty()) plan_p2_tiles(cand, i0, walk, p.rows_x, threads, core + 2 * (rows - p.rows_x), p.tiles_x, p.threads_x);
 }
 
 inline int p2_exact_threads(size_t maxw2) {
diff --git a/wfmash_amd/csrc/wfa_tile2.hip b/wfmash_amd/csrc/wfa_tile2.hip
--- a/wfmash_amd/csrc/wfa_tile2.hip
+++ b/wfmash_amd/csrc/wfa_tile2.hip
@@ -841,15 +841,15 @@
     else hipLaunchKernelGGL((wfa_tile2_kernel<1024, false, false, true>), dim3(ntasks), dim3(threads), lds1, st, pk, ring, jobs, tasks, mak, T, (int32_t*)nullptr, lean);
   }
 }
-void launch_tile2_p2(const uint32_t* pk, int32_t* ring, const TileJob* jobs, const TileTask* tasks, int ntasks, int threads, int32_t* p2, hipStream_t st) {
-  const size_t lds1 = (size_t)(P2K + 1) * 4;
+void launch_tile2_p2(const uint32_t* pk, int32_t* ring, const TileJob* jobs, const TileTask* tasks, int ntasks, int threads, int rows, int32_t* p2, hipStream_t st) {
+  const size_t lds1 = (size_t)(rows + 1) * 4;
   const int lean = tile_lean();
   if (tile_fast()) {
-    if (threads <= 64) hipLaunchKernelGGL((wfa_tile2_kernel<64, true, true, false>), dim3(ntasks), dim3(64), 0, st, pk, ring, jobs, tasks, (int32_t*)nullptr, P2K, p2, lean);
-    else hipLaunchKernelGGL((wfa_tile2_kernel<1024, true, true, false>), dim3(ntasks), dim3(threads), 0, st, pk, ring, jobs, tasks, (int32_t*)nullptr, P2K, p2, lean);
+    if (threads <= 64) hipLaunchKernelGGL((wfa_tile2_kernel<64, true, true, false>), dim3(ntasks), dim3(64), 0, st, pk, ring, jobs, tasks, (int32_t*)nullptr, rows, p2, lean);
+    else hipLaunchKernelGGL((wfa_tile2_kernel<1024, true, true, false>), dim3(ntasks), dim3(threads), 0, st, pk, ring, jobs, tasks, (int32_t*)nullptr, rows, p2, lean);
   } else {
-    if (threads <= 64) hipLaunchKernelGGL((wfa_tile2_kernel<64, true, false, true>), dim3(ntasks), dim3(64), lds1, st, pk, ring, jobs, tasks, (int32_t*)nullptr, P2K, p2, lean);
-    else hipLaunchKernelGGL((wfa_tile2_kernel<1024, true, false, true>), dim3(ntasks), dim3(threads), lds1, st, pk, ring, jobs, tasks, (int32_t*)nullptr, P2K, p2, lean);
+    if (threads <= 64) hipLaunchKernelGGL((wfa_tile2_kernel<64, true, false, true>), dim3(ntasks), dim3(64), lds1, st, pk, ring, jobs, tasks, (int32_t*)nullptr, rows, p2, lean);
+    else hipLaunchKernelGGL((wfa_tile2_kernel<1024, true, false, true>), dim3(ntasks), dim3(threads), lds1, st, pk, ring, jobs, tasks, (int32_t*)nullptr, rows, p2, lean);
   }
 }
 
diff --git a/wfmash_amd/host/capi_host.cpp b/wfmash_amd/host/capi_host.cpp
--- a/wfmash_amd/host/capi_host.cpp
+++ b/wfmash_amd/host/capi_host.cpp
@@ -537,6 +537,22 @@
   return 0;
 }
 
+int wfmh_test_p2_plan_kinds(const int32_t* cand, int64_t n, int64_t i0, int rows, int rows_bm, unsigned long long budget, int threads, int core,
+                            const char* exact, int rows_exact, const int32_t* pen_o, int32_t* tasks, int64_t tasks_cap, int64_t* scalars) {
+  if (i0 < 0 || i0 >= n || rows < 1 || threads < 1 || core < 1 || !exact || !pen_o) return -1;
+  wfm::P2ChunkPlan p;
+  wfm::plan_p2_chunk(reinterpret_cast<const wfm::P2PlanJob*>(cand), (size_t)n, (size_t)i0, rows, rows_bm, (size_t)budget, threads, core, p, exact, rows_exact);
+  const size_t n1 = std::min<size_t>(p.tiles.tasks.size(), (size_t)tasks_cap), n2 = std::min<size_t>(p.tiles_x.tasks.size(), (size_t)tasks_cap - n1);
+  memcpy(tasks, p.tiles.tasks.data(), n1 * sizeof(wfm::TileTask));
+  memcpy(tasks + 4 * n1, p.tiles_x.tasks.data(), n2 * sizeof(wfm::TileTask));
+  wfm_penalties_t pen{};
+  pen.o1 = pen_o[0]; pen.o2 = pen_o[1];
+  const int64_t v[12] = {(int64_t)p.geo.size(), (int64_t)p.elems, p.rows_x, p.threads_c, p.tiles.core_c, (int64_t)p.tiles.tasks.size(), (int64_t)p.tiles.n_pk,
+                         p.threads_x, p.tiles_x.core_c, (int64_t)p.tiles_x.tasks.size(), (int64_t)p.tiles_x.n_pk, wfm::p2_exact_rows(pen)};
+  std::copy(v, v + 12, scalars);
+  return 0;
+}
+
 int wfmh_test_base_plan(int op, const int32_t* in, int64_t n, int32_t* out) {
   if (op == 0) {
     for (int64_t i = 0; i < n; ++i, in += 10)
```

After: 70.52 million aligned bases/s, median of 6. 1.6% higher.
